# DanMcGann/loam

Measured on AMD Instinct MI355X. Metric: scan-pair registrations/sec (64x1024 Ouster), higher is better.
Workload: dtype f64; 1 GPU; batch of 1024 independent 64x1024 scan pairs per GPU (BASELINE configs[2]/[3]); step = extractFeatures x2 + registerFeatures per pair, inputs resident in HBM; pairs_per_gpu=1024, scan=64x1024, seed=20240311, input_scalar=f64, arithmetic=f64 (float input is widened on load)

## Files before the change

include/loamx.h:

```cpp
#ifndef LOAMX_H_
#define LOAMX_H_

#include <stddef.h>
#include <stdint.h>

#ifdef __cplusplus
extern "C" {
#endif

typedef struct loamx_ctx loamx_ctx;

enum {
  LOAMX_OK = 0,
  LOAMX_ERR_SCAN_SIZE = 1,
  LOAMX_ERR_BAD_PARAM = 2,
  LOAMX_ERR_HIP = 3,
  LOAMX_ERR_CAPACITY = 4,
  LOAMX_ERR_UNSUPPORTED = 5,
  LOAMX_ERR_NO_DEVICE = 6,
  LOAMX_ERR_COMM = 7
};

typedef struct {
  uint64_t scan_lines;
// ... 65 lines not shown
int loamx_ctx_synchronize(loamx_ctx* ctx);
int loamx_ctx_extract_counters(loamx_ctx* ctx, uint64_t* tie_replays, uint64_t* scan_fallbacks);
enum {
  LOAMX_ROUTE_SPLIT_CURV = 1u << 0,
  LOAMX_ROUTE_CURV2 = 1u << 1,
  LOAMX_ROUTE_CURV_V1 = 1u << 2,
  LOAMX_ROUTE_CURV_GENERIC = 1u << 3,
  LOAMX_ROUTE_ROWS = 1u << 4,
  LOAMX_ROUTE_ROWS_CH11 = 1u << 5,
  LOAMX_ROUTE_ROWS_PASS2 = 1u << 6,
  LOAMX_ROUTE_ROWS_LIST16 = 1u << 7,
  LOAMX_ROUTE_MIS = 1u << 8,
  LOAMX_ROUTE_MIS_4LINES = 1u << 9,
  LOAMX_ROUTE_MIS_TWO = 1u << 10,
  LOAMX_ROUTE_MIS_CONST_W = 1u << 11,
  LOAMX_ROUTE_ARGMAX4 = 1u << 12,
  LOAMX_ROUTE_ARGMAX1 = 1u << 13,
  LOAMX_ROUTE_FUSED_COMPACT = 1u << 14,
  LOAMX_ROUTE_COMPACT = 1u << 15,
  LOAMX_ROUTE_FUSED_EXTRACT = 1u << 16,
  LOAMX_ROUTE_FUSED_ROWS = 1u << 17,
  LOAMX_ROUTE_BOXES = 1u << 18,
  LOAMX_ROUTE_ROWS_R_SHIFT = 20,
  LOAMX_ROUTE_ROWS_CH_SHIFT = 24
};
int loamx_ctx_last_extract_route(loamx_ctx* ctx, uint32_t* bits);
enum {
  LOAMX_WALK_NONE = 0,
  LOAMX_WALK_FLAT = 1,
  LOAMX_WALK_TILED_BY_COUNT = 2,
  LOAMX_WALK_TILED_BY_TILES = 3
};
typedef struct {
  uint32_t iterations, termination;
  uint32_t use_moments;
  uint32_t mom_ref_on;
  double mom_ref[7];
  uint32_t tiles;
  uint32_t live_tiles;
  uint64_t edge_stride, planar_stride;
  uint32_t n_se, n_sp;
  uint32_t walk;
  uint32_t listed_total;
  double s0max, v2max;
  uint32_t sweep_chunk, edge_cache, list_cache, flat_cache;
  uint32_t* tile_counts;
  size_t tile_counts_cap;
} loamx_solve_census;
int loamx_ctx_last_solve_census(loamx_ctx* ctx, size_t pair, loamx_solve_census* out);
enum { LOAMX_ASSOC_SEARCH_NONE = 0, LOAMX_ASSOC_SEARCH_BRUTE = 1, LOAMX_ASSOC_SEARCH_GRID = 2 };
enum { LOAMX_ASSOC_LEFTOVER_NONE = 0, LOAMX_ASSOC_LEFTOVER_LEFT = 1, LOAMX_ASSOC_LEFTOVER_COOP = 2 };
#define LOAMX_ASSOC_REASON_WIDE 0x80000000u
#define LOAMX_ASSOC_REASON_TIED 0x40000000u
typedef struct {
  uint32_t n_src, n_tgt;
  uint64_t stride;
  uint32_t km;
  uint32_t search;
  uint32_t mixed_launch;
  uint32_t one_stage;
  uint32_t leftover_kernel;
  uint32_t rest_blocks, coop_blocks;
  uint32_t rest_spread, left_spread;
  uint32_t lean_set;
  double origin[3], h;
  int32_t nx, ny, nz;
  uint32_t n_points;
  uint32_t verified, unverified, queued_words;
  uint32_t queued, queued_plain, queued_wide, queued_tied;
  uint32_t rest_searched;
  uint32_t listed;
  uint32_t leftover_finished;
  uint32_t exact;
  uint32_t late;
  uint32_t* entry_query;
  uint32_t* entry_reason;
  int32_t* count_after_rest;
  int32_t* count_before_fit;
  size_t entries_cap;
  uint32_t* late_query;
  size_t late_cap;
} loamx_assoc_census;
int loamx_ctx_last_assoc_census(loamx_ctx* ctx, int which_kind, loamx_assoc_census* out);
int loamx_ctx_set_option(loamx_ctx* ctx, const char* name, int value);
int loamx_ctx_get_option(loamx_ctx* ctx, const char* name, int* value);


int loamx_compute_curvature(loamx_ctx* ctx, const double* xyz, size_t n_points, const loamx_lidar_params* lidar,
                            const loamx_fe_params* fe, double* curvature_out);
int loamx_compute_valid_points(loamx_ctx* ctx, const double* xyz, size_t n_points,
                               const loamx_lidar_params* lidar, const loamx_fe_params* fe, uint8_t* mask_out);
int loamx_extract_features(loamx_ctx* ctx, const double* xyz, size_t n_points, const loamx_lidar_params* lidar,
                           const loamx_fe_params* fe, uint32_t* edge_idx, size_t edge_cap, size_t* n_edge,
                           uint32_t* planar_idx, size_t planar_cap, size_t* n_planar);
int loamx_compute_curvature_f32(loamx_ctx* ctx, const float* xyz, size_t n_points, const loamx_lidar_params* lidar,
                                const loamx_fe_params* fe, double* curvature_out);
int loamx_compute_valid_points_f32(loamx_ctx* ctx, const float* xyz, size_t n_points,
                                   const loamx_lidar_params* lidar, const loamx_fe_params* fe, uint8_t* mask_out);
int loamx_extract_features_f32(loamx_ctx* ctx, const float* xyz, size_t n_points, const loamx_lidar_params* lidar,
                               const loamx_fe_params* fe, uint32_t* edge_idx, size_t edge_cap, size_t* n_edge,
                               uint32_t* planar_idx, size_t planar_cap, size_t* n_planar);
int loamx_register_features(loamx_ctx* ctx, const double* src_edge, size_t n_src_edge, const double* src_planar,
                            size_t n_src_planar, const double* tgt_edge, size_t n_tgt_edge,
                            const double* tgt_planar, size_t n_tgt_planar, const double init_pose[7],
                            const loamx_reg_params* reg, loamx_reg_result* result, loamx_reg_detail* detail);

typedef struct loamx_target_index loamx_target_index;
int loamx_target_index_create(loamx_ctx* ctx, const double* tgt_edge, size_t n_tgt_edge, const double* tgt_planar,
                              size_t n_tgt_planar, const loamx_reg_params* reg, loamx_target_index** out);
void loamx_target_index_destroy(loamx_ctx* ctx, loamx_target_index* index);
int loamx_target_index_insert(loamx_ctx* ctx, loamx_target_index* index, const double* edge, size_t n_edge,
                              const double* planar, size_t n_planar);
int loamx_target_index_stats(const loamx_target_index* index, uint64_t* full_builds, uint64_t* merges);
int loamx_target_index_size(const loamx_target_index* index, size_t* n_edge, size_t* n_planar);
enum {
  LOAMX_INDEX_BUILD_NONE = 0,
  LOAMX_INDEX_BUILD_PACKED = 1,
  LOAMX_INDEX_BUILD_SINGLE = 2,
  LOAMX_INDEX_BUILD_BIG = 3
};
enum { LOAMX_INDEX_OP_NONE = 0, LOAMX_INDEX_OP_FULL_BUILD = 1, LOAMX_INDEX_OP_MERGE = 2 };
typedef struct {
  uint64_t n, capacity;
  double origin[3], h, inv_h;
  int32_t nx, ny, nz;
  uint32_t n_points;
  uint32_t build;
  uint32_t table_valid;
  uint64_t table_entries;
  uint32_t lds_passes;
  uint32_t scan_tiles;
  uint32_t last_op, reserved;
  uint64_t full_builds, merges;
  uint32_t* cell_start;
  size_t cell_start_cap;
  double* xyz;
  uint32_t* orig;
  size_t points_cap;
  float* rel;
  size_t rel_cap;
} loamx_index_census;
int loamx_target_index_census(loamx_ctx* ctx, const loamx_target_index* index, int which_set, loamx_index_census* out);
int loamx_register_features_indexed(loamx_ctx* ctx, const loamx_target_index* index, const double* src_edge,
                                    size_t n_src_edge, const double* src_planar, size_t n_src_planar,
                                    const double init_pose[7], const loamx_reg_params* reg, loamx_reg_result* result,
                                    loamx_reg_detail* detail);


int loamx_target_index_points(loamx_ctx* ctx, const loamx_target_index* index, int which_set, size_t first, size_t count,
                              double* xyz_out);
int loamx_voxel_filter_dev(loamx_ctx* ctx, const double* d_xyz, size_t n, const double pose[7], double leaf, double* d_xyz_out,
                           uint32_t* d_src_idx, uint32_t* d_n_out);
int loamx_target_index_insert_filtered(loamx_ctx* ctx, loamx_target_index* index, const double* edge, size_t n_edge,
                                       const double* planar, size_t n_planar, const double world_T_scan[7], double edge_leaf,
                                       double planar_leaf, size_t* n_edge_added, size_t* n_planar_added);
int loamx_target_index_crop(loamx_ctx* ctx, loamx_target_index* index, const double lo[3], const double hi[3],
                            size_t* n_edge_removed, size_t* n_planar_removed);


int loamx_fit_lines(loamx_ctx* ctx, const double* points, size_t n_sets, size_t k, double* lines_out, double* cond_out);
int loamx_fit_planes(loamx_ctx* ctx, const double* points, size_t n_sets, size_t k, double* planes_out, double* avg_dist_out);
int loamx_knn_search(loamx_ctx* ctx, const loamx_target_index* index, int which_set, const double* queries, size_t n_queries,
                     size_t k, double max_dist, uint32_t* indices_out, uint32_t* counts_out);
typedef struct {
  uint32_t* edge_nn_count;
  uint32_t* edge_nn_idx;
// ... 316 lines not shown
```

loam_amd/capi.py:

```python
import collections
import ctypes as C
import os

import numpy as np

from . import build as _build

OK, ERR_SCAN_SIZE, ERR_BAD_PARAM, ERR_HIP, ERR_CAPACITY, ERR_UNSUPPORTED, ERR_NO_DEVICE, ERR_COMM = range(8)
CONVERGED, MAX_ITER, INSUFFICIENT_ASSOCIATIONS = 0, 1, 2
K_CURVATURE, K_SELECT, K_COMPACT, K_GRID, K_ASSOC, K_SWEEP, K_LM, K_MOMENT, K_KNN_PLANE, K_EXTRACT_FUSED, K_INFORMATION, K_CLOUD_ACCUMULATE, K_CLOUD_ACCUMULATE_PLAIN, K_CLOUD_LIST, K_CLOUD_EMIT, K_COUNT = range(16)


class LidarParams(C.Structure):
    _fields_ = [("scan_lines", C.c_uint64), ("points_per_line", C.c_uint64), ("min_range", C.c_double),
                ("max_range", C.c_double)]


class FeatureExtractionParams(C.Structure):
    _fields_ = [("neighbor_points", C.c_uint64), ("number_sectors", C.c_uint64),
                ("max_edge_feats_per_sector", C.c_uint64), ("max_planar_feats_per_sector", C.c_uint64),
                ("edge_feat_threshold", C.c_double), ("planar_feat_threshold", C.c_double),
                ("occlusion_thresh", C.c_double), ("parallel_thresh", C.c_double)]

    def __init__(self, *a, **kw):
# ... 148 lines not shown
            if not 0 <= getattr(self, name) <= 0xFFFFFFFF:
                raise ValueError(f"PlaceParams: {name} does not fit 32 bits")
        return PlaceParamsStruct(self.n_rings, self.n_sectors, self.max_range, self.z_offset, self.z_scale)


PLACE_MATCH_DTYPE = np.dtype([("id", np.uint32), ("shift", np.uint32), ("key_dist", np.uint64), ("distance", np.float64)])
PLACE_NO_ID = 0xFFFFFFFF


class CloudMapParamsStruct(C.Structure):
    _fields_ = [("leaf", C.c_double), ("min_range", C.c_double), ("max_range", C.c_double)]


class CloudMapParams:

    def __init__(self, leaf=None, min_range=None, max_range=None):
        d = CloudMapParamsStruct()
        load().loamx_default_cloud_map_params(C.byref(d))
        self.leaf = d.leaf if leaf is None else float(leaf)
        self.min_range = d.min_range if min_range is None else float(min_range)
        self.max_range = d.max_range if max_range is None else float(max_range)

    def struct(self):
        return CloudMapParamsStruct(float(self.leaf), float(self.min_range), float(self.max_range))


CLOUD_MAP_STATS_DTYPE = np.dtype([(n, np.uint64) for n in ("voxels", "points_offered", "points_used", "invalid", "range", "outside", "overflow")])


class PgoParamsStruct(C.Structure):
    _fields_ = [("max_iterations", C.c_uint32), ("max_pcg_iterations", C.c_uint32), ("pcg_tolerance", C.c_double),
                ("initial_lambda", C.c_double), ("cost_tolerance", C.c_double), ("step_tolerance", C.c_double),
                ("huber_delta", C.c_double)]


class PgoParams:
    FIELDS = tuple(f[0] for f in PgoParamsStruct._fields_)

    def __init__(self, **kw):
        d = PgoParamsStruct()
        load().loamx_pgo_default_params(C.byref(d))
        for name in self.FIELDS:
            setattr(self, name, getattr(d, name))
        for name, v in kw.items():
            if name not in self.FIELDS:
                raise TypeError(f"PgoParams has no field {name}")
            setattr(self, name, v)

    def struct(self):
        for name in self.FIELDS[:2]:
            if not 0 <= int(getattr(self, name)) <= 0xFFFFFFFF:
                raise ValueError(f"PgoParams: {name} does not fit 32 bits")
        return PgoParamsStruct(int(self.max_iterations), int(self.max_pcg_iterations), *(float(getattr(self, n)) for n in self.FIELDS[2:]))


PGO_EDGE_DTYPE = np.dtype([("a", np.uint32), ("b", np.uint32), ("a_T_b", np.float64, 7), ("information", np.float64, (6, 6))])
PGO_SUMMARY_DTYPE = np.dtype([("initial_cost", np.float64), ("final_cost", np.float64), ("lambda", np.float64), ("max_update", np.float64),
                              ("iterations", np.uint32), ("accepted", np.uint32), ("pcg_iterations", np.uint32),
                              ("termination", np.uint32), ("n_bad_edges", np.uint32), ("reserved", np.uint32)])
PGO_LINEARIZATION_DTYPE = np.dtype([("e", np.float64, 6), ("chi2", np.float64), ("weight", np.float64), ("A", np.float64, (6, 6)),
                                    ("B", np.float64, (6, 6))])
PGO_TERMINATIONS = ("COST_CONVERGED", "STEP_CONVERGED", "MAX_ITERATIONS", "LAMBDA_OVERFLOW", "NOTHING_TO_DO", "BAD_INPUT")
(PGO_COST_CONVERGED, PGO_STEP_CONVERGED, PGO_MAX_ITERATIONS, PGO_LAMBDA_OVERFLOW, PGO_NOTHING_TO_DO, PGO_BAD_INPUT) = range(6)


EXPORTS = [
    "loamx_default_fe_params", "loamx_default_reg_params", "loamx_status_string", "loamx_last_error",
    "loamx_ctx_create", "loamx_ctx_destroy", "loamx_ctx_set_stream", "loamx_ctx_synchronize",
    "loamx_compute_curvature", "loamx_compute_valid_points", "loamx_extract_features", "loamx_register_features",
    "loamx_target_index_create", "loamx_target_index_destroy", "loamx_register_features_indexed",
    "loamx_edge_capacity", "loamx_planar_capacity", "loamx_extract_features_batch_dev",
    "loamx_register_features_batch_dev", "loamx_register_scan_pairs_dev", "loamx_register_scan_pairs",
    "loamx_register_scan_pairs_f32", "loamx_ctx_enable_kernel_timing",
    "loamx_ctx_reset_kernel_stats", "loamx_ctx_get_kernel_stats", "loamx_kernel_name", "loamx_synth_pair_pose",
    "loamx_synth_scan_host", "loamx_synth_scan_pairs_dev", "loamx_dev_alloc", "loamx_dev_free",
    "loamx_copy_to_device", "loamx_copy_to_host",
    "loamx_compute_curvature_f32", "loamx_compute_valid_points_f32", "loamx_extract_features_f32",
    "loamx_extract_features_batch_dev_f32", "loamx_register_scan_pairs_dev_f32",
    "loamx_target_index_insert", "loamx_target_index_size", "loamx_target_index_census",
    "loamx_shard_range", "loamx_comm_get_unique_id", "loamx_comm_create", "loamx_comm_wrap", "loamx_comm_destroy",
    "loamx_comm_info", "loamx_gather_results_dev", "loamx_comm_barrier", "loamx_comm_stats", "loamx_ctx_extract_counters",
    "loamx_ctx_set_option", "loamx_ctx_get_option", "loamx_ctx_last_extract_route", "loamx_ctx_last_solve_census",
    "loamx_ctx_last_assoc_census",
    "loamx_fit_lines", "loamx_fit_planes", "loamx_knn_search", "loamx_associate", "loamx_target_index_stats",
    "loamx_register_scan_sequence_dev", "loamx_register_scan_sequence_dev_f32", "loamx_register_scan_sequence",
    "loamx_register_scan_sequence_f32", "loamx_compose_trajectory_dev", "loamx_deskew_scans_dev", "loamx_deskew_scans_dev_f32",
    "loamx_deskew_launch_geometry",
    "loamx_target_index_points", "loamx_voxel_filter_dev", "loamx_target_index_insert_filtered", "loamx_target_index_crop",
    "loamx_registration_information", "loamx_registration_information_indexed", "loamx_registration_information_batch_dev",
    "loamx_register_scan_pairs_info_dev", "loamx_register_scan_pairs_info_dev_f32", "loamx_register_scan_sequence_info_dev",
    "loamx_register_scan_sequence_info_dev_f32",
    "loamx_default_organize_params", "loamx_scan_layout_create", "loamx_scan_layout_destroy", "loamx_scan_layout_tables",
    "loamx_organize_clouds_dev", "loamx_organize_clouds_dev_f32", "loamx_organize_cloud", "loamx_organize_cloud_f32",
    "loamx_default_place_params", "loamx_place_db_create", "loamx_place_db_destroy", "loamx_place_db_sector_dirs", "loamx_place_db_size",
    "loamx_place_descriptors_dev", "loamx_place_descriptors_dev_f32", "loamx_place_db_add_dev", "loamx_place_db_read",
    "loamx_place_search_dev", "loamx_place_descriptor", "loamx_place_descriptor_f32", "loamx_place_search",
    "loamx_pgo_default_params", "loamx_pose_graph_optimize_dev", "loamx_pose_graph_optimize", "loamx_pose_graph_linearize",
    "loamx_pose_graph_edges_from_results_dev",
    "loamx_default_cloud_map_params", "loamx_cloud_map_create", "loamx_cloud_map_destroy", "loamx_cloud_map_clear",
    "loamx_cloud_map_add_clouds_dev", "loamx_cloud_map_add_clouds_dev_f32", "loamx_cloud_map_emit_dev", "loamx_cloud_map_stats_read",
    "loamx_cloud_map_add_cloud", "loamx_cloud_map_add_cloud_f32", "loamx_cloud_map_emit", "loamx_cloud_map_claims_read",
]

ROUTE_BITS = ("SPLIT_CURV", "CURV2", "CURV_V1", "CURV_GENERIC", "ROWS", "ROWS_CH11", "ROWS_PASS2", "ROWS_LIST16", "MIS", "MIS_4LINES",
              "MIS_TWO", "MIS_CONST_W", "ARGMAX4", "ARGMAX1", "FUSED_COMPACT", "COMPACT", "FUSED_EXTRACT", "FUSED_ROWS", "BOXES")


class ExtractRoute:

    def __init__(self, bits):
        self.bits = int(bits)
        self.names = frozenset(n for i, n in enumerate(ROUTE_BITS) if self.bits >> i & 1)
        self.rows_R = self.bits >> 20 & 7
        self.rows_ch = self.bits >> 24 & 63

    def __contains__(self, name):
        if name not in ROUTE_BITS:
            raise KeyError(name)
        return name in self.names

    def __repr__(self):
        return "ExtractRoute(%s%s)" % ("|".join(n for n in ROUTE_BITS if n in self.names),
                                       ", R=%d ch=%d" % (self.rows_R, self.rows_ch) if "ROWS" in self.names else "")


class SolveCensusStruct(C.Structure):
    _fields_ = [("iterations", C.c_uint32), ("termination", C.c_uint32), ("use_moments", C.c_uint32), ("mom_ref_on", C.c_uint32),
                ("mom_ref", C.c_double * 7), ("tiles", C.c_uint32), ("live_tiles", C.c_uint32),
                ("edge_stride", C.c_uint64), ("planar_stride", C.c_uint64), ("n_se", C.c_uint32), ("n_sp", C.c_uint32),
                ("walk", C.c_uint32), ("listed_total", C.c_uint32), ("s0max", C.c_double), ("v2max", C.c_double),
                ("sweep_chunk", C.c_uint32), ("edge_cache", C.c_uint32), ("list_cache", C.c_uint32), ("flat_cache", C.c_uint32),
                ("tile_counts", C.POINTER(C.c_uint32)), ("tile_counts_cap", C.c_size_t)]


WALK_NONE, WALK_FLAT, WALK_TILED_BY_COUNT, WALK_TILED_BY_TILES = 0, 1, 2, 3
WALK_NAMES = ("none", "flat", "tiled-by-count", "tiled-by-tiles")
SolveCensus = collections.namedtuple(
    "SolveCensus", "iterations termination use_moments mom_ref_on mom_ref tiles live_tiles edge_stride planar_stride n_se n_sp walk "
                   "listed_total s0max v2max sweep_chunk edge_cache list_cache flat_cache tile_counts")


class AssocCensusStruct(C.Structure):
    _fields_ = ([("n_src", C.c_uint32), ("n_tgt", C.c_uint32), ("stride", C.c_uint64)] +
                [(n, C.c_uint32) for n in ("km", "search", "mixed_launch", "one_stage", "leftover_kernel", "rest_blocks", "coop_blocks",
                                           "rest_spread", "left_spread", "lean_set")] +
                [("origin", C.c_double * 3), ("h", C.c_double), ("nx", C.c_int32), ("ny", C.c_int32), ("nz", C.c_int32)] +
                [(n, C.c_uint32) for n in ("n_points", "verified", "unverified", "queued_words", "queued", "queued_plain", "queued_wide",
                                           "queued_tied", "rest_searched", "listed", "leftover_finished", "exact", "late")] +
                [("entry_query", C.POINTER(C.c_uint32)), ("entry_reason", C.POINTER(C.c_uint32)),
                 ("count_after_rest", C.POINTER(C.c_int32)), ("count_before_fit", C.POINTER(C.c_int32)), ("entries_cap", C.c_size_t),
                 ("late_query", C.POINTER(C.c_uint32)), ("late_cap", C.c_size_t)])


ASSOC_SEARCH_NONE, ASSOC_SEARCH_BRUTE, ASSOC_SEARCH_GRID = 0, 1, 2
ASSOC_LEFTOVER_NONE, ASSOC_LEFTOVER_LEFT, ASSOC_LEFTOVER_COOP = 0, 1, 2
ASSOC_REASON_WIDE, ASSOC_REASON_TIED = 0x80000000, 0x40000000
ASSOC_CENSUS_SCALARS = ("n_src n_tgt stride km search mixed_launch one_stage leftover_kernel rest_blocks coop_blocks rest_spread left_spread "
                        "lean_set h nx ny nz n_points verified unverified queued_words queued queued_plain queued_wide queued_tied "
                        "rest_searched listed leftover_finished exact late").split()
AssocCensus = collections.namedtuple("AssocCensus", ASSOC_CENSUS_SCALARS + ["origin", "entry_query", "entry_reason", "count_after_rest",
                                                                            "count_before_fit", "late_query"])


class IndexCensusStruct(C.Structure):
    _fields_ = [("n", C.c_uint64), ("capacity", C.c_uint64), ("origin", C.c_double * 3), ("h", C.c_double), ("inv_h", C.c_double),
                ("nx", C.c_int32), ("ny", C.c_int32), ("nz", C.c_int32), ("n_points", C.c_uint32),
# ... 49 lines not shown
    lib.loamx_compute_valid_points_f32.argtypes = [vp, fp, C.c_size_t, C.POINTER(LidarParams),
                                                   C.POINTER(FeatureExtractionParams), C.POINTER(C.c_uint8)]
    lib.loamx_extract_features_f32.argtypes = [vp, fp, C.c_size_t, C.POINTER(LidarParams),
                                               C.POINTER(FeatureExtractionParams), u32p, C.c_size_t,
                                               C.POINTER(C.c_size_t), u32p, C.c_size_t, C.POINTER(C.c_size_t)]
    lib.loamx_register_features.argtypes = [vp, dp, C.c_size_t, dp, C.c_size_t, dp, C.c_size_t, dp, C.c_size_t, dp,
                                            C.POINTER(RegistrationParams), C.POINTER(RegResult),
                                            C.POINTER(RegDetail)]
    lib.loamx_target_index_create.argtypes = [vp, dp, C.c_size_t, dp, C.c_size_t, C.POINTER(RegistrationParams), C.POINTER(vp)]
    lib.loamx_target_index_insert.argtypes = [vp, vp, dp, C.c_size_t, dp, C.c_size_t]
    lib.loamx_target_index_size.argtypes = [vp, C.POINTER(C.c_size_t), C.POINTER(C.c_size_t)]
    lib.loamx_target_index_stats.argtypes = [vp, C.POINTER(C.c_uint64), C.POINTER(C.c_uint64)]
    lib.loamx_target_index_points.argtypes = [vp, vp, C.c_int, C.c_size_t, C.c_size_t, dp]
    lib.loamx_target_index_census.argtypes = [vp, vp, C.c_int, C.POINTER(IndexCensusStruct)]
    lib.loamx_voxel_filter_dev.argtypes = [vp, vp, C.c_size_t, dp, C.c_double, vp, vp, vp]
    lib.loamx_target_index_insert_filtered.argtypes = [vp, vp, dp, C.c_size_t, dp, C.c_size_t, dp, C.c_double, C.c_double,
                                                       C.POINTER(C.c_size_t), C.POINTER(C.c_size_t)]
    lib.loamx_target_index_crop.argtypes = [vp, vp, dp, dp, C.POINTER(C.c_size_t), C.POINTER(C.c_size_t)]
    lib.loamx_target_index_destroy.argtypes = [vp, vp]
    lib.loamx_target_index_destroy.restype = None
    lib.loamx_register_features_indexed.argtypes = [vp, vp, dp, C.c_size_t, dp, C.c_size_t, dp, C.POINTER(RegistrationParams),
                                                    C.POINTER(RegResult), C.POINTER(RegDetail)]
    lib.loamx_edge_capacity.restype = C.c_size_t
    lib.loamx_edge_capacity.argtypes = [C.POINTER(LidarParams), C.POINTER(FeatureExtractionParams)]
    lib.loamx_planar_capacity.restype = C.c_size_t
    lib.loamx_planar_capacity.argtypes = [C.POINTER(LidarParams), C.POINTER(FeatureExtractionParams)]
    lib.loamx_extract_features_batch_dev.argtypes = [vp, vp, C.c_size_t, C.POINTER(LidarParams),
                                                     C.POINTER(FeatureExtractionParams), vp, vp, vp, vp, vp, vp]
    lib.loamx_extract_features_batch_dev_f32.argtypes = lib.loamx_extract_features_batch_dev.argtypes
    lib.loamx_register_features_batch_dev.argtypes = [vp, C.c_size_t, vp, vp, vp, vp, vp, vp, vp, vp, C.c_size_t,
                                                      C.c_size_t, vp, C.POINTER(RegistrationParams), vp]
    lib.loamx_register_scan_pairs_dev.argtypes = [vp, vp, C.c_size_t, C.POINTER(LidarParams),
                                                  C.POINTER(FeatureExtractionParams), C.POINTER(RegistrationParams),
                                                  vp]
    lib.loamx_register_scan_pairs_dev_f32.argtypes = lib.loamx_register_scan_pairs_dev.argtypes
    lib.loamx_register_scan_pairs.argtypes = lib.loamx_register_scan_pairs_dev.argtypes
    lib.loamx_register_scan_pairs_f32.argtypes = lib.loamx_register_scan_pairs_dev.argtypes
    lib.loamx_register_scan_sequence_dev.argtypes = [vp, vp, C.c_size_t, C.POINTER(LidarParams),
                                                     C.POINTER(FeatureExtractionParams), C.POINTER(RegistrationParams),
                                                     vp, vp]
    lib.loamx_register_scan_sequence_dev_f32.argtypes = lib.loamx_register_scan_sequence_dev.argtypes
    lib.loamx_register_scan_sequence.argtypes = lib.loamx_register_scan_sequence_dev.argtypes
    lib.loamx_register_scan_sequence_f32.argtypes = lib.loamx_register_scan_sequence_dev.argtypes
    lib.loamx_compose_trajectory_dev.argtypes = [vp, vp, C.c_size_t, dp, vp]
    lib.loamx_deskew_scans_dev.argtypes = [vp, vp, C.c_size_t, C.POINTER(LidarParams), vp, C.c_double, vp]
    lib.loamx_deskew_scans_dev_f32.argtypes = lib.loamx_deskew_scans_dev.argtypes
    lib.loamx_deskew_launch_geometry.argtypes = [C.c_size_t, C.c_uint64, C.c_uint64, u32p]
    lib.loamx_ctx_enable_kernel_timing.argtypes = [vp, C.c_int]
    lib.loamx_ctx_reset_kernel_stats.argtypes = [vp]
    lib.loamx_ctx_get_kernel_stats.argtypes = [vp, C.POINTER(KernelStat)]
    lib.loamx_synth_pair_pose.argtypes = [C.c_uint64, C.c_uint64, dp]
    lib.loamx_synth_pair_pose.restype = None
    lib.loamx_synth_scan_host.argtypes = [C.c_uint64, C.c_uint64, C.c_uint32, C.c_uint32, C.c_uint32, C.c_double, dp]
    lib.loamx_synth_scan_host.restype = None
    lib.loamx_synth_scan_pairs_dev.argtypes = [vp, C.c_uint64, C.c_uint64, C.c_size_t, C.c_uint32, C.c_uint32,
                                               C.c_double, vp]
    lib.loamx_dev_alloc.argtypes = [vp, C.c_size_t, C.POINTER(vp)]
    lib.loamx_dev_free.argtypes = [vp, vp]
    lib.loamx_copy_to_device.argtypes = [vp, vp, vp, C.c_size_t]
    lib.loamx_copy_to_host.argtypes = [vp, vp, vp, C.c_size_t]
    szp = C.POINTER(C.c_size_t)
    lib.loamx_shard_range.argtypes = [C.c_size_t, C.c_int, C.c_int, szp, szp]
    lib.loamx_shard_range.restype = None
    lib.loamx_comm_get_unique_id.argtypes = [C.c_char_p]
    lib.loamx_comm_create.argtypes = [vp, C.c_char_p, C.c_int, C.c_int, C.POINTER(vp)]
    lib.loamx_comm_wrap.argtypes = [vp, vp, C.POINTER(vp)]
    lib.loamx_comm_destroy.argtypes = [vp]
    lib.loamx_comm_destroy.restype = None
    lib.loamx_comm_info.argtypes = [vp, C.POINTER(C.c_int), C.POINTER(C.c_int), C.POINTER(C.c_int)]
    lib.loamx_gather_results_dev.argtypes = [vp, vp, vp, C.c_size_t, C.c_size_t, vp]
    lib.loamx_comm_barrier.argtypes = [vp, vp, dp]
    lib.loamx_comm_stats.argtypes = [vp, C.POINTER(C.c_uint64)]
    lib.loamx_ctx_extract_counters.argtypes = [vp, C.POINTER(C.c_uint64), C.POINTER(C.c_uint64)]
    lib.loamx_fit_lines.argtypes = [vp, dp, C.c_size_t, C.c_size_t, dp, dp]
    lib.loamx_fit_planes.argtypes = [vp, dp, C.c_size_t, C.c_size_t, dp, dp]
    lib.loamx_knn_search.argtypes = [vp, vp, C.c_int, dp, C.c_size_t, C.c_size_t, C.c_double, vp, vp]
    lib.loamx_associate.argtypes = [vp, dp, C.c_size_t, dp, C.c_size_t, dp, C.c_size_t, dp, C.c_size_t, dp,
                                    C.POINTER(RegistrationParams), C.POINTER(AssocDump)]
    lib.loamx_ctx_set_option.argtypes = [vp, C.c_char_p, C.c_int]
    lib.loamx_ctx_get_option.argtypes = [vp, C.c_char_p, C.POINTER(C.c_int)]
    lib.loamx_ctx_last_extract_route.argtypes = [vp, C.POINTER(C.c_uint32)]
    lib.loamx_ctx_last_solve_census.argtypes = [vp, C.c_size_t, C.POINTER(SolveCensusStruct)]
    lib.loamx_ctx_last_assoc_census.argtypes = [vp, C.c_int, C.POINTER(AssocCensusStruct)]
    lib.loamx_registration_information.argtypes = [vp, dp, C.c_size_t, dp, C.c_size_t, dp, C.c_size_t, dp, C.c_size_t, dp,
                                                   C.POINTER(RegistrationParams), C.POINTER(RegInformation)]
    lib.loamx_registration_information_indexed.argtypes = [vp, vp, dp, C.c_size_t, dp, C.c_size_t, dp, C.POINTER(RegistrationParams),
                                                           C.POINTER(RegInformation)]
    lib.loamx_registration_information_batch_dev.argtypes = lib.loamx_register_features_batch_dev.argtypes
    lib.loamx_register_scan_pairs_info_dev.argtypes = lib.loamx_register_scan_pairs_dev.argtypes + [vp]
    lib.loamx_register_scan_pairs_info_dev_f32.argtypes = lib.loamx_register_scan_pairs_info_dev.argtypes
    lib.loamx_register_scan_sequence_info_dev.argtypes = lib.loamx_register_scan_sequence_dev.argtypes + [vp]
    lib.loamx_register_scan_sequence_info_dev_f32.argtypes = lib.loamx_register_scan_sequence_info_dev.argtypes
    lib.loamx_default_organize_params.argtypes = [C.POINTER(OrganizeParamsStruct)]
    lib.loamx_default_organize_params.restype = None
    lib.loamx_scan_layout_create.argtypes = [vp, C.POINTER(LidarParams), C.POINTER(OrganizeParamsStruct), C.POINTER(vp)]
    lib.loamx_scan_layout_destroy.argtypes = [vp, vp]
    lib.loamx_scan_layout_destroy.restype = None
    lib.loamx_scan_layout_tables.argtypes = [vp, dp, dp]
    lib.loamx_organize_clouds_dev.argtypes = [vp, vp, vp, C.c_size_t, vp, szp, C.c_size_t, vp, vp, vp]
    lib.loamx_organize_clouds_dev_f32.argtypes = lib.loamx_organize_clouds_dev.argtypes
    lib.loamx_organize_cloud.argtypes = [vp, vp, vp, C.c_size_t, vp, C.c_size_t, vp, vp, vp]
    lib.loamx_organize_cloud_f32.argtypes = lib.loamx_organize_cloud.argtypes
    lib.loamx_default_place_params.argtypes = [C.POINTER(PlaceParamsStruct)]
    lib.loamx_default_place_params.restype = None
    lib.loamx_place_db_create.argtypes = [vp, C.POINTER(PlaceParamsStruct), C.POINTER(vp)]
    lib.loamx_place_db_destroy.argtypes = [vp, vp]
    lib.loamx_place_db_destroy.restype = None
    lib.loamx_place_db_sector_dirs.argtypes = [vp, dp]
    lib.loamx_place_db_size.argtypes = [vp, szp]
    lib.loamx_place_descriptors_dev.argtypes = [vp, vp, vp, C.c_size_t, szp, C.c_size_t, vp]
    lib.loamx_place_descriptors_dev_f32.argtypes = lib.loamx_place_descriptors_dev.argtypes
    lib.loamx_place_db_add_dev.argtypes = [vp, vp, vp, C.c_size_t, u32p]
    lib.loamx_place_db_read.argtypes = [vp, vp, C.c_size_t, C.c_size_t, vp, vp, vp]
    lib.loamx_place_search_dev.argtypes = [vp, vp, vp, C.c_size_t, vp, C.c_uint32, vp]
    lib.loamx_place_descriptor.argtypes = [vp, vp, vp, C.c_size_t, C.c_size_t, vp]
    lib.loamx_place_descriptor_f32.argtypes = lib.loamx_place_descriptor.argtypes
    lib.loamx_place_search.argtypes = lib.loamx_place_search_dev.argtypes
    lib.loamx_default_cloud_map_params.argtypes = [C.POINTER(CloudMapParamsStruct)]
    lib.loamx_default_cloud_map_params.restype = None
    lib.loamx_cloud_map_create.argtypes = [vp, C.POINTER(CloudMapParamsStruct), C.c_size_t, C.POINTER(vp)]
    lib.loamx_cloud_map_destroy.argtypes = [vp, vp]
    lib.loamx_cloud_map_destroy.restype = None
    lib.loamx_cloud_map_clear.argtypes = [vp, vp]
    lib.loamx_cloud_map_add_clouds_dev.argtypes = [vp, vp, vp, C.c_size_t, szp, C.c_size_t, vp]
    lib.loamx_cloud_map_add_clouds_dev_f32.argtypes = lib.loamx_cloud_map_add_clouds_dev.argtypes
    lib.loamx_cloud_map_emit_dev.argtypes = [vp, vp, C.c_uint32, vp, vp, vp, C.c_size_t, vp]
    lib.loamx_cloud_map_stats_read.argtypes = [vp, vp, vp]
    lib.loamx_cloud_map_claims_read.argtypes = [vp, vp, C.POINTER(C.c_uint64)]
    lib.loamx_cloud_map_add_cloud.argtypes = [vp, vp, vp, C.c_size_t, C.c_size_t, vp]
    lib.loamx_cloud_map_add_cloud_f32.argtypes = lib.loamx_cloud_map_add_cloud.argtypes
    lib.loamx_cloud_map_emit.argtypes = [vp, vp, C.c_uint32, vp, vp, vp, C.c_size_t, szp]
    lib.loamx_pgo_default_params.argtypes = [C.POINTER(PgoParamsStruct)]
    lib.loamx_pgo_default_params.restype = None
    lib.loamx_pose_graph_optimize_dev.argtypes = [vp, vp, C.c_size_t, vp, vp, C.c_size_t, C.POINTER(PgoParamsStruct), vp]
    lib.loamx_pose_graph_optimize.argtypes = lib.loamx_pose_graph_optimize_dev.argtypes
    lib.loamx_pose_graph_linearize.argtypes = [vp, vp, C.c_size_t, vp, C.c_size_t, C.c_double, vp]
    lib.loamx_pose_graph_edges_from_results_dev.argtypes = [vp, vp, vp, C.c_size_t, C.c_uint32, vp]
    _lib = lib
    return lib


class LoamxError(RuntimeError):
    def __init__(self, status, message):
        super().__init__(message)
        self.status = status


DeskewGeometry = collections.namedtuple("DeskewGeometry", "col_blocks shares lines_per_share unroll")


def deskew_launch_geometry(n_scans, scan_lines, points_per_line):
    v = (C.c_uint32 * 4)()
    rc = load().loamx_deskew_launch_geometry(n_scans, scan_lines, points_per_line, v)
    if rc != OK:
        raise LoamxError(rc, "loamx_deskew_launch_geometry: " + load().loamx_status_string(rc).decode())
    return DeskewGeometry(*(int(x) for x in v))


def _dp(a):
    return a.ctypes.data_as(C.POINTER(C.c_double))


def _pts(a):
    a = np.ascontiguousarray(np.asarray(a, dtype=np.float64).reshape(-1, 3))
    return a

# ... 319 lines not shown
        p = C.c_void_p()
        ctx._check(ctx.lib.loamx_dev_alloc(ctx.h, nbytes, C.byref(p)))
        self.ptr = p.value

    def upload(self, arr):
        arr = np.ascontiguousarray(arr)
        assert arr.nbytes <= self.nbytes
        self.ctx._check(self.ctx.lib.loamx_copy_to_device(self.ctx.h, self.ptr, arr.ctypes.data, arr.nbytes))
        return self

    def download(self, dtype, count):
        out = np.empty(count, dtype=dtype)
        assert out.nbytes <= self.nbytes
        self.ctx._check(self.ctx.lib.loamx_copy_to_host(self.ctx.h, out.ctypes.data, self.ptr, out.nbytes))
        return out

    def free(self):
        if self.ptr:
            self.ctx.lib.loamx_dev_free(self.ctx.h, self.ptr)
            self.ptr = None


class Context:

    def __init__(self, device=0):
        self.lib = load()
        h = C.c_void_p()
        rc = self.lib.loamx_ctx_create(device, C.byref(h))
        if rc != OK:
            raise LoamxError(rc, "loamx_ctx_create: " + self.lib.loamx_status_string(rc).decode() +
                             " (libloamx has no CPU fallback)")
        self.h = h

    def close(self):
        if getattr(self, "h", None):
            self.lib.loamx_ctx_destroy(self.h)
            self.h = None

    def __del__(self):
        try:
            self.close()
        except Exception:
            pass

    def _check(self, rc):
        if rc != OK:
            msg = self.lib.loamx_last_error(self.h).decode() or self.lib.loamx_status_string(rc).decode()
            raise LoamxError(rc, msg)

    def set_stream(self, hip_stream_handle):
        self._check(self.lib.loamx_ctx_set_stream(self.h, hip_stream_handle))

    def synchronize(self):
        self._check(self.lib.loamx_ctx_synchronize(self.h))

    def set_option(self, name, value=1):
        self._check(self.lib.loamx_ctx_set_option(self.h, name.encode(), int(value)))

    def get_option(self, name):
        v = C.c_int(0)
        self._check(self.lib.loamx_ctx_get_option(self.h, name.encode(), C.byref(v)))
        return v.value

    def extract_counters(self):
        a, b = C.c_uint64(0), C.c_uint64(0)
        self._check(self.lib.loamx_ctx_extract_counters(self.h, C.byref(a), C.byref(b)))
        return a.value, b.value

    def last_extract_route(self):
        v = C.c_uint32(0)
        self._check(self.lib.loamx_ctx_last_extract_route(self.h, C.byref(v)))
        return ExtractRoute(v.value)

    def last_solve_census(self, pair=0):
        v = SolveCensusStruct()
        self._check(self.lib.loamx_ctx_last_solve_census(self.h, pair, C.byref(v)))
        counts = np.zeros(max(1, v.live_tiles), dtype=np.uint32)
        v.tile_counts, v.tile_counts_cap = counts.ctypes.data_as(C.POINTER(C.c_uint32)), v.live_tiles
        self._check(self.lib.loamx_ctx_last_solve_census(self.h, pair, C.byref(v)))
        return SolveCensus(v.iterations, v.termination, v.use_moments, v.mom_ref_on, np.array(list(v.mom_ref)), v.tiles, v.live_tiles,
                           v.edge_stride, v.planar_stride, v.n_se, v.n_sp, v.walk, v.listed_total, v.s0max, v.v2max, v.sweep_chunk,
                           v.edge_cache, v.list_cache, v.flat_cache, counts[:v.live_tiles].copy())

    def last_assoc_census(self, kind):
        kind = {"edge": 0, "plane": 1}.get(kind, kind)
        v = AssocCensusStruct()
        self._check(self.lib.loamx_ctx_last_assoc_census(self.h, kind, C.byref(v)))
        q = int(v.queued)
        eq, er = np.zeros(max(1, q), dtype=np.uint32), np.zeros(max(1, q), dtype=np.uint32)
        ar, bf = np.zeros(max(1, q), dtype=np.int32), np.zeros(max(1, q), dtype=np.int32)
        v.entry_query, v.entry_reason = eq.ctypes.data_as(C.POINTER(C.c_uint32)), er.ctypes.data_as(C.POINTER(C.c_uint32))
        v.count_after_rest, v.count_before_fit = ar.ctypes.data_as(C.POINTER(C.c_int32)), bf.ctypes.data_as(C.POINTER(C.c_int32))
        v.entries_cap = q
        nl = int(v.late)
        lq = np.zeros(max(1, nl), dtype=np.uint32)
        v.late_query, v.late_cap = lq.ctypes.data_as(C.POINTER(C.c_uint32)), nl
        self._check(self.lib.loamx_ctx_last_assoc_census(self.h, kind, C.byref(v)))
        return AssocCensus(*[getattr(v, n) for n in ASSOC_CENSUS_SCALARS], np.array(list(v.origin)), eq[:q].copy(), er[:q].copy(),
                           ar[:q].copy(), bf[:q].copy(), lq[:nl].copy())

    def alloc(self, nbytes):
        return DeviceBuffer(self, nbytes)

    def compute_curvature(self, xyz, lidar, fe=None):
        fe = fe or FeatureExtractionParams()
        xyz = _scan(xyz)
        out = np.empty(len(xyz))
        fn = self.lib.loamx_compute_curvature_f32 if xyz.dtype == np.float32 else self.lib.loamx_compute_curvature
        self._check(fn(self.h, _xyzp(xyz), len(xyz), C.byref(lidar), C.byref(fe), _dp(out)))
        return out

    def compute_valid_points(self, xyz, lidar, fe=None):
        fe = fe or FeatureExtractionParams()
        xyz = _scan(xyz)
        out = np.empty(len(xyz), dtype=np.uint8)
        fn = self.lib.loamx_compute_valid_points_f32 if xyz.dtype == np.float32 else self.lib.loamx_compute_valid_points
        self._check(fn(self.h, _xyzp(xyz), len(xyz), C.byref(lidar), C.byref(fe), out.ctypes.data_as(C.POINTER(C.c_uint8))))
        return out.astype(bool)

    def extract_features(self, xyz, lidar, fe=None):
        fe = fe or FeatureExtractionParams()
        xyz = _scan(xyz)
        ecap = max(1, self.lib.loamx_edge_capacity(C.byref(lidar), C.byref(fe)))
        pcap = max(1, self.lib.loamx_planar_capacity(C.byref(lidar), C.byref(fe)))
        e = np.empty(ecap, dtype=np.uint32)
        p = np.empty(pcap, dtype=np.uint32)
        ne, npl = C.c_size_t(0), C.c_size_t(0)
        u32p = C.POINTER(C.c_uint32)
        fn = self.lib.loamx_extract_features_f32 if xyz.dtype == np.float32 else self.lib.loamx_extract_features
        self._check(fn(self.h, _xyzp(xyz), len(xyz), C.byref(lidar), C.byref(fe), e.ctypes.data_as(u32p), ecap, C.byref(ne),
                       p.ctypes.data_as(u32p), pcap, C.byref(npl)))
        return e[:ne.value].copy(), p[:npl.value].copy()

    def register_features(self, src_edge, src_planar, tgt_edge, tgt_planar, init_pose=None, reg=None,
                          want_detail=False):
        reg = reg or RegistrationParams()
        arrs = [_pts(a) for a in (src_edge, src_planar, tgt_edge, tgt_planar)]
        init = np.ascontiguousarray([0, 0, 0, 1, 0, 0, 0] if init_pose is None else init_pose, dtype=np.float64)
        res = RegResult()
        detail = None
        if want_detail:
            mi = max(1, reg.max_iterations)
            info = (IterInfo * mi)()
            ce, cp = max(1, len(arrs[0])), max(1, len(arrs[1]))
            ep = np.zeros((mi, ce, 2), dtype=np.uint32)
            pp = np.zeros((mi, cp, 2), dtype=np.uint32)
            nep = np.zeros(mi, dtype=np.uint32)
            npp = np.zeros(mi, dtype=np.uint32)
            u32p = C.POINTER(C.c_uint32)
            detail = RegDetail(info, 0, ep.ctypes.data_as(u32p), ce, nep.ctypes.data_as(u32p),
                               pp.ctypes.data_as(u32p), cp, npp.ctypes.data_as(u32p))
        self._check(self.lib.loamx_register_features(
            self.h, _dp(arrs[0]), len(arrs[0]), _dp(arrs[1]), len(arrs[1]), _dp(arrs[2]), len(arrs[2]),
            _dp(arrs[3]), len(arrs[3]), _dp(init), C.byref(reg), C.byref(res),
            C.byref(detail) if detail is not None else None))
        pose = np.array(list(res.pose))
        if want_detail:
            d = dict(iterations=[dict(target_T_source_init=np.array(list(info[i].target_T_source_init)),
                                      estimate_update=np.array(list(info[i].estimate_update)),
                                      n_edge=info[i].n_edge_associations, n_plane=info[i].n_plane_associations,
                                      edge_pairs=ep[i, :nep[i]].copy(), plane_pairs=pp[i, :npp[i]].copy())
                                 for i in range(detail.n_iter_info)])
            return pose, res.termination, res.iterations, d
        return pose, res.termination, res.iterations

    def fit_lines(self, points):
# ... 394 lines not shown
```

loam_amd/csrc/api_core.hip:

```cpp
#include "api_host.h"
#include "synth.h"

using namespace loamx;

namespace loamx {
thread_local LaunchScope* g_launch_scope = nullptr;
int g_debug_sync = getenv("LOAMX_DEBUG_SYNC") ? 1 : 0;
thread_local uint32_t g_extract_route = 0;
}

namespace {

const char* kKernelNames[LOAMX_K_COUNT] = {"curvature_valid_kernel", "select_kernel", "compact_kernel",
                                           "grid_build_kernel",      "associate_kernel", "sweep_kernel",
                                           "lm_kernels",             "moment_kernel",    "knn_plane_kernel",
                                           "extract_fused_kernel",   "information_kernel", "cloud_accumulate_kernel",
                                           "cloud_accumulate_plain_kernel", "cloud_list_kernels", "cloud_emit_kernels"};

struct OptionName {
  const char* name;
  bool extract;
  uint32_t bit;
};
const OptionName kOptionNames[] = {
    {"FORCE_TIE_REPLAY", true, kFlagForceReplay}, {"FORCE_SCAN_GIVEUP", true, kFlagForceGiveUp}, {"CURV_V1", true, kFlagCurvV1},
    {"NO_FUSED_COMPACT", true, kFlagNoFusedCompact}, {"NO_MIS_SELECT", true, kFlagNoMisSelect}, {"FUSED_EXTRACT", true, kFlagFusedExtract},
    {"NO_ROW_SELECT", true, kFlagNoRowSelect}, {"FUSED_ROWS", true, kFlagFusedRows}, {"NO_SPLIT_CURV", true, kFlagNoSplitCurv}, {"STAGE_ALWAYS", true, kFlagStageAlways},
    {"NO_MOMENTS", false, kRegFlagNoMoments}, {"NO_PACKED_GRID", false, kRegFlagNoPackedGrid}, {"NO_BIG_GRID", false, kRegFlagNoBigGrid},
    {"NO_GRID_SIDE", false, kRegFlagNoGridSide}, {"DEBUG_POISON", false, kRegFlagPoison},
    {"QUEUE_TWO_STAGE", false, kRegFlagQueueTwoStage}, {"QUEUE_ONE_STAGE", false, kRegFlagQueueOneStage},
    {"NO_MIXED_ASSOC", false, kRegFlagNoMixedAssoc}, {"FORCE_RCCL", false, kRegFlagForceRccl},
    {"NO_COOP_LEFT", false, kRegFlagNoCoopLeft}, {"NO_REF_MOMENTS", false, kRegFlagNoRefMoments},
    {"NO_EXTRACT_BOXES", false, kRegFlagNoExtractBoxes}, {"CHECK_FINITE", false, kRegFlagCheckFinite},
    {"NO_SMALL_SETS", false, kRegFlagNoSmallSets}, {"FORCE_LATE_VERIFY", false, kRegFlagForceLate},
    {"NO_LIVE_DEAL", false, kRegFlagNoLiveDeal}, {"NO_CLOUDMAP_COMBINE", false, kRegFlagNoCloudmapCombine}};

}

namespace loamx {

int fail(loamx_ctx* ctx, int code, const std::string& msg) {
  if (ctx) ctx->last_error = msg;
  return code;
}

int ensure(loamx_ctx* ctx, Buf& b, size_t bytes) {
  if (bytes == 0) bytes = 8;
  if (b.cap >= bytes) return LOAMX_OK;
  if (b.p) {
    HIP_TRY(ctx, hipStreamSynchronize(ctx->stream));
    HIP_TRY(ctx, hipFree(b.p));
    b.p = nullptr, b.cap = 0;
  }
  HIP_TRY(ctx, hipMalloc(&b.p, bytes));
  b.cap = bytes;
  return LOAMX_OK;
}
int ensure(loamx_ctx* ctx, int id, size_t bytes) { return ensure(ctx, ctx->ws[id], bytes); }

const char* const kNonFiniteMsg = "non-finite coordinate in the input (the reference's behaviour is undefined there)";
bool host_all_finite(const void* p, bool f32, size_t n_scalars) {
  if (!p) return true;
  if (f32) {
    const float* v = static_cast<const float*>(p);
    float acc = 0.0f;
    for (size_t i = 0; i < n_scalars; i++) acc += v[i] * 0.0f;
    return acc == 0.0f;
  }
  const double* v = static_cast<const double*>(p);
  double acc = 0.0;
  for (size_t i = 0; i < n_scalars; i++) acc += v[i] * 0.0;
  return acc == 0.0;
}

hipEvent_t take_event(loamx_ctx* ctx) {
  if (!ctx->event_pool.empty()) {
    hipEvent_t e = ctx->event_pool.back();
    ctx->event_pool.pop_back();
    return e;
  }
  hipEvent_t e = nullptr;
  (void)hipEventCreate(&e);
  return e;
}

int finite_begin(loamx_ctx* ctx) {
  ENSURE(ctx, WS_FINITE_FLAG, 16);
  untimed(ctx);
  HIP_TRY(ctx, hipMemsetAsync(ctx->ws[WS_FINITE_FLAG].p, 0, 16, ctx->stream));
  return LOAMX_OK;
}
void finite_add(loamx_ctx* ctx, const void* d_pts, bool f32, const uint32_t* d_n, size_t n_sets, size_t stride, uint32_t pitch) {
  if (d_pts && n_sets && stride) launch_check_finite(d_pts, f32, d_n, n_sets, stride, pitch, static_cast<uint32_t*>(ctx->ws[WS_FINITE_FLAG].p), ctx->stream);
}
int finite_end(loamx_ctx* ctx) {
  uint32_t bad = 0;
  HIP_TRY(ctx, hipMemcpyAsync(&bad, ctx->ws[WS_FINITE_FLAG].p, 4, hipMemcpyDeviceToHost, ctx->stream));
  HIP_TRY(ctx, hipStreamSynchronize(ctx->stream));
  return bad ? fail(ctx, LOAMX_ERR_BAD_PARAM, kNonFiniteMsg) : LOAMX_OK;
}
int dev_check_finite(loamx_ctx* ctx, const void* d_pts, bool f32, const uint32_t* d_n, size_t n_sets, size_t stride, uint32_t pitch, bool force) {
  if ((!force && !(ctx->reg_flags & kRegFlagCheckFinite)) || !d_pts || n_sets == 0 || stride == 0) return LOAMX_OK;
  int rc = finite_begin(ctx);
  if (rc != LOAMX_OK) return rc;
  finite_add(ctx, d_pts, f32, d_n, n_sets, stride, pitch);
  return finite_end(ctx);
}

int check_finite_scalars(loamx_ctx* ctx, const double* d, size_t n) {
  int rc = finite_begin(ctx);
  if (rc != LOAMX_OK) return rc;
  launch_check_finite_scalars(d, n, static_cast<uint32_t*>(ctx->ws[WS_FINITE_FLAG].p), ctx->stream);
  return finite_end(ctx);
}

// ... 367 lines not shown
```

loam_amd/csrc/api_host.h:

```cpp
#pragma once
#include <math.h>
#include <stdio.h>
#include <stdlib.h>
#include <string.h>

#include <mutex>
#include <string>
#include <type_traits>
#include <utility>
#include <vector>

#include "loamx_internal.h"

namespace loamx {

enum WsId {
  WS_XYZ = 0, WS_CURV, WS_MASK,
  WS_SORT_SCRATCH, WS_SORT_SCRATCH_SRC, WS_NASSOC, WS_STATE, WS_PARTIALS, WS_MOM_PARTIALS, WS_MOMENTS, WS_FLAGGED_LIST, WS_FLAGGED_COUNT,
  WS_LINE_TOT, WS_EXTRACT_EVENTS, WS_BOX, WS_FINITE_FLAG, WS_COUNTERS, WS_ITERINFO, WS_STREAM_IN0, WS_STREAM_IN1, WS_STREAM_RES,
  WS_FIT_IN, WS_FIT_OUT, WS_FCOUNTS, WS_RESULTS, WS_INIT, WS_STREAM_INIT,
  WS_VOX_TABLE, WS_MAP_WORDS, WS_INFO_PARTIALS, WS_INFO, WS_LIVE,
  WS_ORG_WINNER, WS_ORG_RANGE, WS_ORG_CELL, WS_ORG_COUNTS, WS_ORG_IN, WS_ORG_RINGS, WS_ORG_OUT,
  WS_PLACE_TABLE, WS_PLACE_QKEYS, WS_PLACE_QNORMS, WS_PLACE_CAND_A, WS_PLACE_CAND_B, WS_PLACE_MATCH, WS_PLACE_IN, WS_PLACE_OUT,
  WS_PGO_WORK, WS_PGO_POSES, WS_PGO_FIXED, WS_PGO_EDGES, WS_PGO_OUT,
  WS_CLOUD_IN, WS_CLOUD_POSE, WS_CLOUD_OUT,
  WS_COUNT
};
enum WsKindId {
  WSK_STAGE = 0, WSK_CNT, WSK_IDX, WSK_N, WSK_XYZ,
  WSK_GRID_DESC, WSK_CELLS, WSK_SORTED, WSK_REL, WSK_SGRID_DESC, WSK_SCELLS, WSK_SSORTED, WSK_ASSOC, WSK_NN, WSK_RNN, WSK_NEAREST,
  WSK_REST, WSK_EXACT, WSK_DUMP, WSK_SRC, WSK_TGT, WSK_MAP_TMP, WSK_MAP_OUT, WSK_CENSUS,
  WSK_COUNT
};

struct Buf {
  void* p = nullptr;
  size_t cap = 0;
};

struct PendingEvent {
  int kernel;
  hipEvent_t e0, e1;
  double bytes;
  bool own_e0;
};

}

struct loamx_ctx {
  int device = 0;
  hipStream_t own_stream = nullptr, stream = nullptr;
  bool max_counts_clean = false;
  hipStream_t aux_stream = nullptr;
  hipEvent_t ev_fork = nullptr, ev_mid = nullptr, ev_join = nullptr;
  hipEvent_t ev_counts = nullptr;
  hipStream_t aux2_stream = nullptr;
  hipEvent_t ev_join2 = nullptr;
  std::string last_error;
  loamx::Buf ws[loamx::WS_COUNT];
  loamx::Buf wsk[loamx::WSK_COUNT][2];
  uint32_t* h_pinned = nullptr;
  bool timing = false;
  std::vector<loamx::PendingEvent> pending;
  std::vector<hipEvent_t> event_pool;
  hipEvent_t tail_event = nullptr;
  bool tail_fresh = false;
  loamx_kernel_stat stats[LOAMX_K_COUNT] = {};

  uint32_t extract_flags = 0;
  uint32_t reg_flags = 0;
  int map_cells_log2 = 0;
  int stream_chunk_pairs = 0;
  hipStream_t copy_stream = nullptr;
  hipEvent_t ev_up[2] = {nullptr, nullptr}, ev_free[2] = {nullptr, nullptr};

  uint32_t last_extract_route = 0;
  loamx::RegBatch last_solve_batch = {};
  uint32_t last_solve_flags = 0;
  bool last_solve_valid = false;
  struct AssocCensusKept {
    loamx_assoc_census c;
    std::vector<uint32_t> entry;
    std::vector<int32_t> after_rest, before_fit;
    std::vector<uint32_t> late;
  } last_assoc_census[2];
  bool last_assoc_census_valid = false;

  unsigned long long sweep_slots_base[2] = {0, 0};
  unsigned long long features_base = 0;
  std::mutex mu;
};

struct loamx_target_index {
  loamx::GridDesc* desc[2] = {nullptr, nullptr};
  uint32_t* cells[2] = {nullptr, nullptr};
  loamx::GridPoint* sorted[2] = {nullptr, nullptr};
  float* rel[2] = {nullptr, nullptr};
  double* pts[2] = {nullptr, nullptr};
  size_t n[2] = {0, 0};
  size_t cap[2] = {0, 0};
  double radius[2] = {0, 0};
  uint32_t* counts = nullptr;
  void* scratch = nullptr;
  uint32_t cells_cap[2] = {0, 0};
  size_t cells_alloc[2] = {0, 0}, scratch_alloc = 0;
  loamx::GridPoint* sorted2[2] = {nullptr, nullptr};
  float* rel2[2] = {nullptr, nullptr};
  size_t n_at_build[2] = {0, 0};
  bool grid_valid[2] = {false, false};
  uint64_t full_builds = 0, merges = 0;
  loamx::GridBuildForm build_form[2] = {{0u, 0u, 0u}, {0u, 0u, 0u}};
  bool table_valid[2] = {false, false};
  uint32_t last_op[2] = {0u, 0u};
  uint64_t kind_builds[2] = {0, 0}, kind_merges[2] = {0, 0};
  loamx::VoxelTable vox[2] = {{nullptr, nullptr, 0u}, {nullptr, nullptr, 0u}};
  double vox_leaf[2] = {0, 0};
  size_t vox_n[2] = {0, 0};
  bool vox_valid[2] = {false, false};
};

namespace loamx {

int fail(loamx_ctx* ctx, int code, const std::string& msg);

#define HIP_TRY(ctx, expr)                                                                          \
  do {                                                                                              \
    hipError_t e_ = (expr);                                                                         \
    if (e_ != hipSuccess)                                                                           \
      return fail(ctx, LOAMX_ERR_HIP, std::string(#expr) + ": " + hipGetErrorString(e_));           \
  } while (0)

int ensure(loamx_ctx* ctx, Buf& b, size_t bytes);
int ensure(loamx_ctx* ctx, int id, size_t bytes);
#define ENSURE(ctx, id, bytes)                       \
  do {                                               \
    int rc_ = ensure(ctx, id, bytes);                \
    if (rc_ != LOAMX_OK) return rc_;                 \
  } while (0)

template <typename T>
T* wsp(loamx_ctx* ctx, int id) {
  return reinterpret_cast<T*>(ctx->ws[id].p);
}
template <typename T>
T* wskp(loamx_ctx* ctx, int id, int kind) {
  return reinterpret_cast<T*>(ctx->wsk[id][kind].p);
}

int check_launch(loamx_ctx* ctx, const char* what);
#define CHECK_LAUNCH(ctx, what)                      \
  do {                                               \
    int rc_ = check_launch(ctx, what);               \
    if (rc_ != LOAMX_OK) return rc_;                 \
  } while (0)

struct ApiLock {
  std::lock_guard<std::mutex> guard;
  explicit ApiLock(loamx_ctx* ctx) : guard(ctx->mu) {}
};
#define API_LOCK(ctx)                                \
  if (!ctx) return LOAMX_ERR_BAD_PARAM;              \
  loamx::ApiLock api_lock_(ctx)
#define API_ENTER(ctx)                               \
  API_LOCK(ctx);                                     \
  HIP_TRY(ctx, hipSetDevice(ctx->device))

hipEvent_t take_event(loamx_ctx* ctx);
// ... 98 lines not shown
```

loam_amd/csrc/api_register.hip:

```cpp
#include "api_host.h"

using namespace loamx;

namespace {

int enqueue_association(loamx_ctx* ctx, const RegBatch& B, const RegConfig& C, uint32_t what = kAssocEdges | kAssocPlanes,
                        AssocCensusRun* census = nullptr) {
  hipStream_t s = ctx->stream;
  {
    TimedScope t(ctx, LOAMX_K_ASSOC, 0.0);
    const bool side = (size_t)B.n_pairs * B.kind[kPlane].assoc_blocks >= 128;
    PendingEvent knn{};
    LaunchScope knn_ls{nullptr, nullptr, true};
    if (ctx->timing) {
      knn.kernel = LOAMX_K_KNN_PLANE, knn.bytes = 0.0, knn.own_e0 = true;
      knn.e0 = take_event(ctx), knn.e1 = take_event(ctx);
      knn_ls = LaunchScope{knn.e0, knn.e1, true};
    }
    launch_associate(B, C, s, side ? ctx->aux_stream : nullptr, side ? ctx->aux2_stream : nullptr, ctx->ev_fork, ctx->ev_mid, ctx->ev_join,
                     ctx->ev_join2, ctx->timing ? &knn_ls : nullptr, what, census);
    if (ctx->timing) {
      if (knn_ls.first) ctx->event_pool.push_back(knn.e0), ctx->event_pool.push_back(knn.e1);
      else ctx->pending.push_back(knn);
    }
// ... 163 lines not shown

  if (prebuilt) {
    for (int k = 0; k < 2; k++) B.kind[k].grid = index_grid_set(prebuilt, k);
  }
  {
    TimedScope t(ctx, LOAMX_K_GRID, 0.0);
    const bool side = !(C.flags & kRegFlagNoGridSide) && ctx->aux_stream && !prebuilt && hipStreamWaitEvent(ctx->aux_stream, ctx->ev_counts, 0) == hipSuccess;
    if (!prebuilt) launch_grid_build_targets(B, C, s);
    launch_grid_build_sources(B, C, side ? ctx->aux_stream : s);
    if (side && hipEventRecord(ctx->ev_join, ctx->aux_stream) == hipSuccess) (void)hipStreamWaitEvent(s, ctx->ev_join, 0);
  }
  CHECK_LAUNCH(ctx, "grid_build_kernel");
  HIP_TRY(ctx, hipEventSynchronize(ctx->ev_counts));
  for (int k = 0; k < 2; k++) {
    B.kind[k].assoc_blocks = (ctx->h_pinned[16 + k] + 255u) / 256u;
    const uint32_t tmax = prebuilt ? (uint32_t)prebuilt->n[k] : ctx->h_pinned[18 + k], tmin = prebuilt ? tmax : ctx->h_pinned[20 + k];
    B.kind[k].knn_mode = tmin > tmax ? 0u : (tmin > kBruteMax ? 1u : (tmax <= kBruteMax ? 2u : 0u));
  }
  return LOAMX_OK;
}

int reg_dump(loamx_ctx* ctx, const RegBatch& B, const RegConfig& C, const loamx_assoc_dump* dump, const size_t n_src[2]) {
  if (B.n_pairs == 0) return LOAMX_OK;
  hipStream_t s = ctx->stream;
  if (B.n_pairs != 1) return fail(ctx, LOAMX_ERR_BAD_PARAM, "association dump: one pair at a time");
  RegBatch Bd = B;
  Bd.want_nn_counts = 1u;
  AssocCensusRun census = {};
  for (int kind = 0; kind < 2; kind++) {
    const size_t st = B.kind[kind].stride, bytes = 8 * sizeof(uint32_t) + 2 * st * sizeof(int32_t);
    ENSURE(ctx, ctx->wsk[WSK_CENSUS][kind], bytes);
    HIP_TRY(ctx, hipMemsetAsync(ctx->wsk[WSK_CENSUS][kind].p, 0, bytes, s));
    census.buf[kind].counts = wskp<uint32_t>(ctx, WSK_CENSUS, kind);
    census.buf[kind].after_rest = reinterpret_cast<int32_t*>(census.buf[kind].counts + 8);
    census.buf[kind].before_fit = census.buf[kind].after_rest + st;
  }
  int rc_a = enqueue_association(ctx, Bd, C, kAssocEdges | kAssocPlanes, &census);
  if (rc_a != LOAMX_OK) return rc_a;
  untimed(ctx);
  const size_t n[2] = {n_src[kEdge], n_src[kPlane]}, kq[2] = {(size_t)C.kind[kEdge].k, (size_t)C.kind[kPlane].k}, pw[2] = {6, 4};
  AssocDumpSet D[2] = {};
  for (int kind = 0; kind < 2; kind++) {
    const size_t bytes = n[kind] * (24 + 8 * pw[kind] + 4 + 4 * kq[kind] + 1) + 64;
    ENSURE(ctx, ctx->wsk[WSK_DUMP][kind], bytes);
    unsigned char* base = wskp<unsigned char>(ctx, WSK_DUMP, kind);
    HIP_TRY(ctx, hipMemsetAsync(base, 0, bytes, s));
    D[kind].moved = reinterpret_cast<double*>(base);
    D[kind].prim = D[kind].moved + 3 * n[kind];
    D[kind].nn_count = reinterpret_cast<uint32_t*>(D[kind].prim + pw[kind] * n[kind]);
    D[kind].nn_idx = D[kind].nn_count + n[kind];
    D[kind].valid = reinterpret_cast<uint8_t*>(D[kind].nn_idx + kq[kind] * n[kind]);
    if (n[kind] == 0) D[kind].nn_count = nullptr;
  }
  launch_assoc_dump(B, C, D, s);
  CHECK_LAUNCH(ctx, "assoc_dump_kernel");
  struct Out { void* host; const void* dev; size_t bytes; };
  const Out outs[10] = {
      {dump->edge_nn_count, D[0].nn_count, 4 * n[0]}, {dump->edge_nn_idx, D[0].nn_idx, 4 * kq[0] * n[0]}, {dump->edge_valid, D[0].valid, n[0]},
      {dump->edge_moved, D[0].moved, 24 * n[0]}, {dump->edge_lines, D[0].prim, 48 * n[0]},
      {dump->plane_nn_count, D[1].nn_count, 4 * n[1]}, {dump->plane_nn_idx, D[1].nn_idx, 4 * kq[1] * n[1]}, {dump->plane_valid, D[1].valid, n[1]},
      {dump->plane_moved, D[1].moved, 24 * n[1]}, {dump->plane_planes, D[1].prim, 32 * n[1]}};
  for (const Out& o : outs)
    if (o.host && o.bytes && o.dev) HIP_TRY(ctx, hipMemcpyAsync(o.host, o.dev, o.bytes, hipMemcpyDeviceToHost, s));
  if (dump->queue_lengths) HIP_TRY(ctx, hipMemcpyAsync(dump->queue_lengths, B.n_assoc + 2, 4 * sizeof(uint32_t), hipMemcpyDeviceToHost, s));
  HIP_TRY(ctx, hipStreamSynchronize(s));
  uint32_t na[8];
  HIP_TRY(ctx, hipMemcpy(na, B.n_assoc, sizeof(na), hipMemcpyDeviceToHost));
  for (int kind = 0; kind < 2; kind++) {
    const RegKind& K = B.kind[kind];
    const AssocCensusForm& F = census.form[kind];
    loamx_ctx::AssocCensusKept& keep = ctx->last_assoc_census[kind];
    loamx_assoc_census& c = keep.c;
    c = loamx_assoc_census{};
    GridDesc g;
    uint32_t counts[8];
    HIP_TRY(ctx, hipMemcpy(&g, K.grid.desc, sizeof(g), hipMemcpyDeviceToHost));
    if (F.km == 0u) g = GridDesc{};
    HIP_TRY(ctx, hipMemcpy(counts, census.buf[kind].counts, sizeof(counts), hipMemcpyDeviceToHost));
    c.n_src = (uint32_t)(n[kind] < K.stride ? n[kind] : K.stride), c.n_tgt = g.n_points, c.stride = K.stride;
    c.km = F.km, c.search = F.search, c.mixed_launch = F.mixed_launch, c.one_stage = F.one_stage, c.leftover_kernel = F.leftover_kernel;
    c.rest_blocks = F.rest_blocks, c.coop_blocks = F.coop_blocks;
    c.origin[0] = g.ox, c.origin[1] = g.oy, c.origin[2] = g.oz, c.h = g.h, c.nx = g.nx, c.ny = g.ny, c.nz = g.nz, c.n_points = g.n_points;
    c.verified = counts[0], c.unverified = counts[1], c.queued_words = counts[2];
    c.queued = na[2 + kind], c.listed = na[4 + kind], c.exact = counts[4], c.leftover_finished = counts[3] - counts[4], c.late = na[6 + kind];
    const uint32_t q = c.queued < K.stride ? c.queued : (uint32_t)K.stride;
    keep.entry.assign(q, 0u), keep.after_rest.assign(q, 0), keep.before_fit.assign(q, 0);
    if (q) {
      HIP_TRY(ctx, hipMemcpy(keep.entry.data(), K.rest, q * sizeof(uint32_t), hipMemcpyDeviceToHost));
      HIP_TRY(ctx, hipMemcpy(keep.after_rest.data(), census.buf[kind].after_rest, q * sizeof(int32_t), hipMemcpyDeviceToHost));
      HIP_TRY(ctx, hipMemcpy(keep.before_fit.data(), census.buf[kind].before_fit, q * sizeof(int32_t), hipMemcpyDeviceToHost));
    }
    uint32_t derived[4];
    assoc_census_derive(F, B.n_pairs, g, keep.entry.data(), q, na[4 + kind], derived);
    c.rest_spread = derived[0], c.left_spread = derived[1], c.lean_set = derived[2], c.rest_searched = derived[3];
    const uint32_t nl = c.late < K.stride ? c.late : (uint32_t)K.stride;
    keep.late.assign(nl, 0u);
    if (nl) HIP_TRY(ctx, hipMemcpy(keep.late.data(), K.exact + (K.stride - nl), nl * sizeof(uint32_t), hipMemcpyDeviceToHost));
    if (q || nl) {
      std::vector<GridPoint> sorted(c.n_src);
      HIP_TRY(ctx, hipMemcpy(sorted.data(), K.src_grid.sorted, (size_t)c.n_src * sizeof(GridPoint), hipMemcpyDeviceToHost));
      for (uint32_t t = 0; t < q; t++) {
        const uint32_t i = keep.entry[t] & 0x3FFFFFFFu;
        keep.entry[t] = (keep.entry[t] & ~0x3FFFFFFFu) | (i < c.n_src ? (sorted[i].orig & 0x3FFFFFFFu) : 0x3FFFFFFFu);
      }
      std::vector<uint32_t> tail(keep.late);
      for (uint32_t t = 0; t < nl; t++) {
        const uint32_t i = tail[nl - 1 - t];
        keep.late[t] = i < c.n_src ? sorted[i].orig : 0xFFFFFFFFu;
      }
    }
    for (uint32_t t = 0; t < q; t++) {
      if (keep.entry[t] & LOAMX_ASSOC_REASON_WIDE) c.queued_wide++;
      else if (keep.entry[t] & LOAMX_ASSOC_REASON_TIED) c.queued_tied++;
      else c.queued_plain++;
    }
  }
  ctx->last_assoc_census_valid = true;
  return LOAMX_OK;
}

int reg_information(loamx_ctx* ctx, const RegBatch& B, const RegConfig& C, InfoPartial* info_partials, loamx_reg_information* d_info, bool activate) {
  if (B.n_pairs == 0) return LOAMX_OK;
  hipStream_t s = ctx->stream;
  untimed(ctx);
  if (activate) launch_info_activate(B, s);
  const int rc_a = enqueue_association(ctx, B, C);
  if (rc_a != LOAMX_OK) return rc_a;
  {
    TimedScope t(ctx, LOAMX_K_INFORMATION, 0.0, true);
    launch_information(B, info_partials, d_info, s);
  }
  CHECK_LAUNCH(ctx, "information_kernel");
  return LOAMX_OK;
}

int reg_solve(loamx_ctx* ctx, const RegBatch& B, const RegConfig& C, loamx_reg_result* d_results, AfterAssocHook hook, void* hook_user) {
  if (B.n_pairs == 0) return LOAMX_OK;
  hipStream_t s = ctx->stream;
  ctx->last_solve_batch = B, ctx->last_solve_flags = C.flags, ctx->last_solve_valid = true;
  for (uint32_t it = 0; it < C.max_iterations; it++) {
    {
      const int rc_body = enqueue_icf_iteration(ctx, B, C, it, hook, hook_user);
      if (rc_body != LOAMX_OK) return rc_body;
    }
    if (it + 1 < C.max_iterations && it > (B.n_pairs >= 256 ? 1u : 0u)) {
      untimed(ctx);
      HIP_TRY(ctx, hipMemcpyAsync(ctx->h_pinned, B.live_count(it), sizeof(uint32_t), hipMemcpyDeviceToHost, s));
      launch_write_results(B, d_results, s);
      CHECK_LAUNCH(ctx, "write_results_kernel");
      HIP_TRY(ctx, hipStreamSynchronize(s));
      if (ctx->h_pinned[0] == 0) {
        ctx->max_counts_clean = true;
        return LOAMX_OK;
      }
    }
  }
  untimed(ctx);
  launch_write_results(B, d_results, s);
  CHECK_LAUNCH(ctx, "write_results_kernel");
  ctx->max_counts_clean = true;
  return LOAMX_OK;
}

}

namespace {
// ... 147 lines not shown
}

int loamx_registration_information(loamx_ctx* ctx, const double* src_edge, size_t n_se, const double* src_planar, size_t n_sp,
                                   const double* tgt_edge, size_t n_te, const double* tgt_planar, size_t n_tp, const double pose[7],
                                   const loamx_reg_params* reg, loamx_reg_information* info) {
  if (!info) return LOAMX_ERR_BAD_PARAM;
  return register_features_impl(ctx, nullptr, {{src_edge, src_planar}, {n_se, n_sp}}, {{tgt_edge, tgt_planar}, {n_te, n_tp}}, pose, reg,
                                HostOutput::to_info(info));
}

int loamx_registration_information_indexed(loamx_ctx* ctx, const loamx_target_index* index, const double* src_edge, size_t n_se,
                                           const double* src_planar, size_t n_sp, const double pose[7], const loamx_reg_params* reg,
                                           loamx_reg_information* info) {
  if (!index || !info) return LOAMX_ERR_BAD_PARAM;
  return register_features_impl(ctx, index, {{src_edge, src_planar}, {n_se, n_sp}}, {{nullptr, nullptr}, {0, 0}}, pose, reg,
                                HostOutput::to_info(info));
}

int loamx_ctx_last_solve_census(loamx_ctx* ctx, size_t pair, loamx_solve_census* out) {
  if (!out) return LOAMX_ERR_BAD_PARAM;
  API_ENTER(ctx);
  if (!ctx->last_solve_valid) return fail(ctx, LOAMX_ERR_BAD_PARAM, "no registration on this context to read (or its workspace has been handed on since)");
  const RegBatch& B = ctx->last_solve_batch;
  if (pair >= B.n_pairs) return fail(ctx, LOAMX_ERR_BAD_PARAM, "pair out of range");
  hipStream_t s = ctx->stream;
  untimed(ctx);
  HIP_TRY(ctx, hipStreamSynchronize(s));
  PairState S;
  uint32_t n_raw[2] = {0, 0};
  HIP_TRY(ctx, hipMemcpy(&S, B.state + pair, sizeof(S), hipMemcpyDeviceToHost));
  for (int k = 0; k < 2; k++) HIP_TRY(ctx, hipMemcpy(&n_raw[k], B.kind[k].n_src + pair * B.in_pitch, sizeof(uint32_t), hipMemcpyDeviceToHost));
  uint32_t* const counts_out = out->tile_counts;
  const size_t cap = counts_out ? out->tile_counts_cap : 0;
  *out = loamx_solve_census{};
  out->tile_counts = counts_out, out->tile_counts_cap = cap;
  out->iterations = S.iterations, out->termination = S.termination, out->use_moments = S.use_moments, out->mom_ref_on = S.mom_ref_on;
  for (int i = 0; i < 7; i++) out->mom_ref[i] = S.mom_ref[i];
  out->tiles = B.mom_blocks_per_pair * 4;
  out->edge_stride = B.kind[kEdge].stride, out->planar_stride = B.kind[kPlane].stride;
  out->n_se = n_raw[kEdge] < B.kind[kEdge].stride ? n_raw[kEdge] : (uint32_t)B.kind[kEdge].stride;
  out->n_sp = n_raw[kPlane] < B.kind[kPlane].stride ? n_raw[kPlane] : (uint32_t)B.kind[kPlane].stride;
  out->sweep_chunk = (uint32_t)kSweepChunk, out->edge_cache = kEdgeCache, out->list_cache = kListCache, out->flat_cache = kFlatCache;
  uint32_t live = 0;
  while (live < out->tiles && (size_t)(live / 4) * kSweepChunk < out->n_sp) live++;
  out->live_tiles = live;
  const bool lists = !(ctx->last_solve_flags & kRegFlagNoMoments) && (S.iterations >= 2u || S.mom_ref_on != 0u);
  if (!lists) return LOAMX_OK;
  double maxima[2];
  HIP_TRY(ctx, hipMemcpy(maxima, B.moments + pair * (size_t)(kMomSize + 2) + kMomSize, sizeof(maxima), hipMemcpyDeviceToHost));
  out->s0max = maxima[0], out->v2max = maxima[1];
  std::vector<uint32_t> cnt(live);
  if (live) HIP_TRY(ctx, hipMemcpy(cnt.data(), B.flagged_count + pair * (size_t)out->tiles, live * sizeof(uint32_t), hipMemcpyDeviceToHost));
  for (uint32_t t = 0; t < live; t++) {
    out->listed_total += cnt[t];
    if (t < cap) counts_out[t] = cnt[t];
  }
  out->walk = out->tiles > kListCache ? LOAMX_WALK_TILED_BY_TILES : (out->listed_total > kFlatCache ? LOAMX_WALK_TILED_BY_COUNT : LOAMX_WALK_FLAT);
  return LOAMX_OK;
}

int loamx_ctx_last_assoc_census(loamx_ctx* ctx, int which_kind, loamx_assoc_census* out) {
  if (!out) return LOAMX_ERR_BAD_PARAM;
  API_LOCK(ctx);
  if (which_kind != 0 && which_kind != 1) return fail(ctx, LOAMX_ERR_BAD_PARAM, "which_kind: 0 = edges, 1 = planes");
  if (!ctx->last_assoc_census_valid) return fail(ctx, LOAMX_ERR_BAD_PARAM, "no association dump on this context to read (or another call came after it)");
  const loamx_ctx::AssocCensusKept& keep = ctx->last_assoc_census[which_kind];
  uint32_t *const eq = out->entry_query, *const er = out->entry_reason;
  int32_t *const ar = out->count_after_rest, *const bf = out->count_before_fit;
  const size_t cap = out->entries_cap, lcap = out->late_cap;
  uint32_t* const lq = out->late_query;
  *out = keep.c;
  out->late_query = lq, out->late_cap = lcap;
  for (size_t t = 0; lq && t < keep.late.size() && t < lcap; t++) lq[t] = keep.late[t];
  out->entry_query = eq, out->entry_reason = er, out->count_after_rest = ar, out->count_before_fit = bf, out->entries_cap = cap;
  for (size_t t = 0; t < keep.entry.size() && t < cap; t++) {
    if (eq) eq[t] = keep.entry[t] & 0x3FFFFFFFu;
    if (er) er[t] = keep.entry[t] & (LOAMX_ASSOC_REASON_WIDE | LOAMX_ASSOC_REASON_TIED);
    if (ar) ar[t] = keep.after_rest[t];
    if (bf) bf[t] = keep.before_fit[t];
  }
  return LOAMX_OK;
}

int loamx_associate(loamx_ctx* ctx, const double* src_edge, size_t n_se, const double* src_planar, size_t n_sp, const double* tgt_edge,
                    size_t n_te, const double* tgt_planar, size_t n_tp, const double pose[7], const loamx_reg_params* reg,
                    loamx_assoc_dump* out) {
  if (!out) return LOAMX_ERR_BAD_PARAM;
  return register_features_impl(ctx, nullptr, {{src_edge, src_planar}, {n_se, n_sp}}, {{tgt_edge, tgt_planar}, {n_te, n_tp}}, pose, reg,
                                HostOutput::to_dump(out));
}

static int fit_sets(loamx_ctx* ctx, bool plane, const double* points, size_t n_sets, size_t k, double* prim_out, double* aux_out) {
  API_ENTER(ctx);
  if (n_sets == 0) return LOAMX_OK;
  if (!points || !prim_out) return fail(ctx, LOAMX_ERR_BAD_PARAM, "null argument");
  if (k < (plane ? 3u : 2u)) return fail(ctx, LOAMX_ERR_BAD_PARAM, plane ? "fitPlane needs k >= 3 points" : "fitLine needs k >= 2 points");
  if (k > (size_t)kFitMaxK) return fail(ctx, LOAMX_ERR_UNSUPPORTED, "point sets of more than 32 points are not supported by the fit kernels");
  if (n_sets > 0x7FFFFFFFull / 64) return fail(ctx, LOAMX_ERR_UNSUPPORTED, "too many point sets in one call");
  const size_t pw = plane ? 4 : 6;
  untimed(ctx);
  ENSURE(ctx, WS_FIT_IN, n_sets * k * 24);
  ENSURE(ctx, WS_FIT_OUT, n_sets * (pw + 1) * sizeof(double));
  double* d_prim = wsp<double>(ctx, WS_FIT_OUT);
  double* d_aux = d_prim + n_sets * pw;
  hipStream_t s = ctx->stream;
  HIP_TRY(ctx, hipMemcpyAsync(ctx->ws[WS_FIT_IN].p, points, n_sets * k * 24, hipMemcpyHostToDevice, s));
  {
    int rc = dev_check_finite(ctx, ctx->ws[WS_FIT_IN].p, false, nullptr, 1, n_sets * k, 1, true);
    if (rc != LOAMX_OK) return rc;
  }
  launch_fit_sets(plane, wsp<double>(ctx, WS_FIT_IN), n_sets, (int)k, d_prim, d_aux, s);
  CHECK_LAUNCH(ctx, "fit_sets_kernel");
  HIP_TRY(ctx, hipMemcpyAsync(prim_out, d_prim, n_sets * pw * sizeof(double), hipMemcpyDeviceToHost, s));
  if (aux_out) HIP_TRY(ctx, hipMemcpyAsync(aux_out, d_aux, n_sets * sizeof(double), hipMemcpyDeviceToHost, s));
  HIP_TRY(ctx, hipStreamSynchronize(s));
  return LOAMX_OK;
}

int loamx_fit_lines(loamx_ctx* ctx, const double* points, size_t n_sets, size_t k, double* lines_out, double* cond_out) {
  return fit_sets(ctx, false, points, n_sets, k, lines_out, cond_out);
}
int loamx_fit_planes(loamx_ctx* ctx, const double* points, size_t n_sets, size_t k, double* planes_out, double* avg_dist_out) {
  return fit_sets(ctx, true, points, n_sets, k, planes_out, avg_dist_out);
}

int loamx_knn_search(loamx_ctx* ctx, const loamx_target_index* index, int which_set, const double* queries, size_t n_queries, size_t k,
                     double max_dist, uint32_t* indices_out, uint32_t* counts_out) {
  if (!ctx || !index) return LOAMX_ERR_BAD_PARAM;
  API_ENTER(ctx);
  if (which_set != 0 && which_set != 1) return fail(ctx, LOAMX_ERR_BAD_PARAM, "which_set: 0 = edge points, 1 = planar points");
  if (index->n[which_set] != 0 && !index->grid_valid[which_set])
    return fail(ctx, LOAMX_ERR_BAD_PARAM, "the target index is inconsistent (an insert into it failed): insert again or build a new one");
  if (n_queries == 0) return LOAMX_OK;
  if (!queries || !indices_out || !counts_out) return fail(ctx, LOAMX_ERR_BAD_PARAM, "null argument");
  if (k == 0) {
    memset(counts_out, 0, n_queries * sizeof(uint32_t));
    return LOAMX_OK;
  }
  if (k > (size_t)kMaxK) return fail(ctx, LOAMX_ERR_UNSUPPORTED, "k > 16 neighbours not supported by the search kernels");
  if (n_queries > 0x7FFFFFFFull / 64) return fail(ctx, LOAMX_ERR_UNSUPPORTED, "too many queries in one call");
  untimed(ctx);
  ENSURE(ctx, WS_FIT_IN, n_queries * 24);
  ENSURE(ctx, WS_FIT_OUT, n_queries * (k + 1) * sizeof(uint32_t));
  uint32_t* d_idx = wsp<uint32_t>(ctx, WS_FIT_OUT);
  uint32_t* d_cnt = d_idx + n_queries * k;
  hipStream_t s = ctx->stream;
  HIP_TRY(ctx, hipMemcpyAsync(ctx->ws[WS_FIT_IN].p, queries, n_queries * 24, hipMemcpyHostToDevice, s));
  {
    int rc = dev_check_finite(ctx, ctx->ws[WS_FIT_IN].p, false, nullptr, 1, n_queries, 1, true);
    if (rc != LOAMX_OK) return rc;
  }
  launch_knn_queries(index_grid_set(index, which_set), wsp<double>(ctx, WS_FIT_IN), n_queries, (int)k, max_dist, d_idx, d_cnt, s);
  CHECK_LAUNCH(ctx, "knn_queries_kernel");
  HIP_TRY(ctx, hipMemcpyAsync(indices_out, d_idx, n_queries * k * sizeof(uint32_t), hipMemcpyDeviceToHost, s));
  HIP_TRY(ctx, hipMemcpyAsync(counts_out, d_cnt, n_queries * sizeof(uint32_t), hipMemcpyDeviceToHost, s));
  HIP_TRY(ctx, hipStreamSynchronize(s));
  return LOAMX_OK;
}

static int register_features_batch(loamx_ctx* ctx, size_t n_pairs, const double* d_src_edge, const uint32_t* d_n_src_edge,
                                   const double* d_src_planar, const uint32_t* d_n_src_planar, const double* d_tgt_edge,
                                   const uint32_t* d_n_tgt_edge, const double* d_tgt_planar, const uint32_t* d_n_tgt_planar,
                                   size_t edge_stride, size_t planar_stride, const double* d_init, const loamx_reg_params* reg,
                                   loamx_reg_result* d_results, loamx_reg_information* d_info) {
  API_ENTER(ctx);
  RegConfig C;
// ... 54 lines not shown
```

loam_amd/csrc/loamx_internal.h:

```cpp
#pragma once
#include <hip/hip_runtime.h>
#include <hip/hip_ext.h>
#include <stdint.h>
#include <stdio.h>

#include "../../include/loamx.h"
#include "extract_math.h"
#include "reg_math.h"
#include "organize_math.h"
#include "place_math.h"
#include "xcd_map.h"

namespace loamx {

struct LaunchScope {
  hipEvent_t start, stop;
  bool first;
};
extern thread_local LaunchScope* g_launch_scope;
extern int g_debug_sync;
template <typename F, typename... Args>
inline void launch_kernel_named(const char* name, F kernel, const dim3& grid, const dim3& block, size_t shmem, hipStream_t s, Args... args) {
  LaunchScope* sc = g_launch_scope;
  if (g_debug_sync) fprintf(stderr, "[loamx] launch %s grid %u x %u block %u\n", name, grid.x, grid.y, block.x), fflush(stderr);
// ... 13 lines not shown
constexpr int kMaxNeighborPoints = 16;
constexpr int kMaxLineWidth = 4096;

extern thread_local uint32_t g_extract_route;

struct ExtractStage {
  uint32_t* edge_stage;
  uint32_t* planar_stage;
  uint32_t* edge_cnt;
  uint32_t* planar_cnt;
};

struct ExtractFused {
  unsigned long long* line_tot;
  uint32_t fuse;
  const void* xyz;
  uint32_t f32;
  uint32_t* edge_idx;
  uint32_t* n_edge;
  double* edge_xyz;
  size_t edge_stride;
  uint32_t* planar_idx;
  uint32_t* n_planar;
  double* planar_xyz;
  size_t planar_stride;
  uint32_t* error;
  unsigned long long* events;
  unsigned long long* box_min;
  unsigned long long* box_max;
  uint32_t no_stage;
  const uint32_t* only_if;
};
__device__ __forceinline__ unsigned long long dbl_key(double v) {
  const unsigned long long u = (unsigned long long)__double_as_longlong(v);
  return (u >> 63) ? ~u : (u | 0x8000000000000000ull);
}
__device__ __forceinline__ double key_dbl(unsigned long long k) {
  return __longlong_as_double((long long)((k >> 63) ? (k & 0x7FFFFFFFFFFFFFFFull) : ~k));
}

void launch_curvature_valid(const void* d_xyz, bool f32, size_t n_scans, const ExtractParams& P, double* d_curv,
                            uint8_t* d_mask, hipStream_t s);
bool launch_select(const double* d_curv, const uint8_t* d_mask, size_t n_scans, const ExtractParams& P,
                   const ExtractStage& st, const ExtractFused* fz, hipStream_t s, bool* rows_ran = nullptr);
bool launch_select_takes_boxes(const ExtractParams& P);
bool launch_extract_fused(const void* d_xyz, bool f32, size_t n_scans, const ExtractParams& P, const ExtractStage& st,
                          const ExtractFused& fz, double* d_curv, uint8_t* d_mask, hipStream_t s);
bool launch_extract_rows_fused(const void* d_xyz, bool f32, size_t n_scans, const ExtractParams& P, const ExtractStage& st,
                               const ExtractFused& fz, double* d_curv, uint8_t* d_mask, hipStream_t s);
bool launch_extract_split_ok(const ExtractParams& P, size_t n_scans);
void launch_extract_init(unsigned long long* line_tot, size_t n_tot, unsigned long long* box_min, unsigned long long* box_max, size_t n_box,
                         hipStream_t s);
void launch_replay(const double* d_curv, const uint8_t* d_mask, size_t n_scans, const ExtractParams& P, const ExtractStage& st,
                   const ExtractFused& fz, hipStream_t s);
void launch_compact(const void* d_xyz, bool f32, size_t n_scans, const ExtractParams& P, const ExtractStage& st,
                    uint32_t* d_edge_idx, uint32_t* d_n_edge, double* d_edge_xyz, size_t edge_stride,
                    uint32_t* d_planar_idx, uint32_t* d_n_planar, double* d_planar_xyz, size_t planar_stride,
                    hipStream_t s, const uint32_t* only_if = nullptr, unsigned long long* fallback_counter = nullptr);

constexpr int kEdge = 0, kPlane = 1;
struct RegKindConfig {
  int k;
  double r;
  int min_pts;
  double pass;
};
struct RegConfig {
  RegKindConfig kind[2];
  double min_line_cond, max_avg_plane_dist;
  uint32_t max_iterations;
  double rot_thresh, pos_thresh;
  uint32_t min_associations;
  uint32_t flags;
};
constexpr uint32_t kRegFlagNoMoments = 1u;
constexpr uint32_t kRegFlagNoPackedGrid = 2u;
constexpr uint32_t kRegFlagNoBigGrid = 4u;
constexpr uint32_t kRegFlagNoGridSide = 8u;
constexpr uint32_t kRegFlagPoison = 16u;
constexpr uint32_t kRegFlagQueueTwoStage = 32u;
constexpr uint32_t kRegFlagQueueOneStage = 64u;
constexpr uint32_t kRegFlagForceRccl = 256u;
constexpr uint32_t kRegFlagNoCoopLeft = 512u;
constexpr uint32_t kRegFlagNoRefMoments = 1024u;
constexpr uint32_t kRegFlagNoSmallSets = 8192u;
constexpr uint32_t kRegFlagCheckFinite = 4096u;
constexpr uint32_t kRegFlagNoExtractBoxes = 2048u;
constexpr uint32_t kRegFlagNoMixedAssoc = 128u;
constexpr uint32_t kRegFlagNoLiveDeal = 32768u;
constexpr uint32_t kRegFlagForceLate = 16384u;

struct GridSet {
  GridDesc* desc;
  uint32_t* cell_start;
  GridPoint* sorted;
  size_t stride;
  float* rel;
  uint32_t cells_cap;
};

struct RegKind {
  size_t stride;
  const double* src;
  const uint32_t* n_src;
  const double* tgt;
  const uint32_t* n_tgt;
  GridSet grid;
  GridSet src_grid;
  uint32_t knn_mode;
  uint32_t assoc_blocks;
  double* rec;
  uint32_t* nn;
  uint32_t* rnn;
  uint32_t* nearest;
  uint32_t* rest;
  uint32_t* exact;
};

struct LiveLists {
  uint32_t iter;
  uint32_t n[2];
  uint32_t stamp[2];
  uint32_t pad[3];
};
constexpr uint32_t kLiveFirstIter = 2u;

struct PairState {
  double est[7];
  LmState lm;
  uint32_t active;
  uint32_t termination;
  uint32_t iterations;
  uint32_t first_sweep;
  uint32_t stream_planes;
  uint32_t use_moments;
  uint32_t mom_ref_on;
  double mom_ref[7];
};

constexpr int kSweepThreads = 256;
#ifndef LOAMX_SWEEP_ITEMS
#define LOAMX_SWEEP_ITEMS 16
#endif
constexpr int kSweepItems = LOAMX_SWEEP_ITEMS;
constexpr int kSweepChunk = kSweepThreads * kSweepItems;
constexpr uint32_t kEdgeCache = 320;
constexpr uint32_t kListCache = 64;
constexpr uint32_t kFlatCache = 192;

struct RegBatch {
  size_t n_pairs;
  uint32_t in_pitch;
  RegKind kind[2];
  const double* init;
  GridPoint* sort_scratch;
  GridPoint* sort_scratch_src;
  uint32_t* n_assoc;
  PairState* state;
  double* partials;
  double* mom_partials;
  double* moments;
  uint32_t mom_blocks_per_pair;
  uint32_t* flagged_list;
  uint32_t* flagged_count;
  uint32_t blocks_per_pair;
  uint32_t* n_active;
// ... 211 lines not shown
```

loam_amd/csrc/reg_math.h:

```cpp
#pragma once
#include <stdint.h>

#if defined(__HIPCC__)
#include <hip/hip_runtime.h>
#include <math.h>
#define LOAMX_HD __host__ __device__ __forceinline__
#else
#include <math.h>
#define LOAMX_HD inline
#endif

namespace loamx {

constexpr int kMaxK = 16;
constexpr double kDblMin = 2.2250738585072014e-308;
constexpr double kDblMax = 1.7976931348623157e308;
constexpr double kDblEps = 2.220446049250313e-16;

struct Vec3 {
  double x, y, z;
};
LOAMX_HD Vec3 v3(double x, double y, double z) { return Vec3{x, y, z}; }
LOAMX_HD Vec3 vadd(Vec3 a, Vec3 b) { return Vec3{a.x + b.x, a.y + b.y, a.z + b.z}; }
LOAMX_HD Vec3 vsub(Vec3 a, Vec3 b) { return Vec3{a.x - b.x, a.y - b.y, a.z - b.z}; }
// ... 701 lines not shown
  if (out > 1) return false;
  const double r2 = knn_radius_bound(max_dist);
  double sy2m = slab_dist(q.y, g.oy, g.h, cy - 1), sy2p = slab_dist(q.y, g.oy, g.h, cy + 1);
  double sz2m = slab_dist(q.z, g.oz, g.h, cz - 1), sz2p = slab_dist(q.z, g.oz, g.h, cz + 1);
  sy2m *= sy2m, sy2p *= sy2p, sz2m *= sz2m, sz2p *= sz2p;
  const int32_t xa = cx - 1 < 0 ? 0 : cx - 1, xb = cx + 1 > g.nx - 1 ? g.nx - 1 : cx + 1;
  uint32_t rb[9], re[9];
#pragma unroll
  for (int j = 0; j < 9; j++) {
    const int32_t iy = cy + (j % 3) - 1, iz = cz + (j / 3) - 1;
    const bool ok = xa <= xb && iy >= 0 && iy <= g.ny - 1 && iz >= 0 && iz <= g.nz - 1;
    const uint32_t row = ok ? (uint32_t)((iz * g.ny + iy) * g.nx) : 0u;
    rb[j] = ok ? cell_start_at(cell_start, row + (uint32_t)xa) : 0u;
    re[j] = ok ? cell_start_at(cell_start, row + (uint32_t)xb + 1u) : 0u;
  }
  uint32_t pre[10];
  pre[0] = 0u;
#pragma unroll
  for (int j = 0; j < 9; j++) {
    const double sy2 = j % 3 == 0 ? sy2m : (j % 3 == 1 ? 0.0 : sy2p), sz2 = j / 3 == 0 ? sz2m : (j / 3 == 1 ? 0.0 : sz2p);
    const bool in_reach = sy2 + sz2 <= r2;
    pre[j + 1] = pre[j] + ((in_reach && rb[j] < re[j]) ? re[j] - rb[j] : 0u);
  }
  const uint32_t total = pre[9];
  if (total > kRow16Cap) return false;
  KnnResult<KM> mine[NL];
#pragma unroll
  for (int v = 0; v < NL; v++) knn_init(mine[v]);
  for (uint32_t base = 0; base < total; base += (uint32_t)(kRow16Lanes * kRow16Batch)) {
#pragma unroll
    for (int v = 0; v < NL; v++) {
      uint32_t at[kRow16Batch];
      bool real[kRow16Batch];
#pragma unroll
      for (int u = 0; u < kRow16Batch; u++) {
        const uint32_t n = base + (uint32_t)(lane0 + v) + (uint32_t)(u * kRow16Lanes);
        real[u] = n < total;
        uint32_t p = 0u;
#pragma unroll
        for (int j = 0; j < 9; j++)
          if (n >= pre[j] && n < pre[j + 1]) p = rb[j] + (n - pre[j]);
        at[u] = p;
      }
      GridPoint t[kRow16Batch];
#pragma unroll
      for (int u = 0; u < kRow16Batch; u++)
        t[u] = *reinterpret_cast<const GridPoint*>(reinterpret_cast<const char*>(sp) + (uint32_t)(at[u] << 5));
#pragma unroll
      for (int u = 0; u < kRow16Batch; u++) {
        const double dx = q.x - t[u].x, dy = q.y - t[u].y, dz = q.z - t[u].z;
        const double d2 = dx * dx + dy * dy + dz * dz;
        if (real[u] && d2 <= mine[v].worst) knn_insert(mine[v], k, d2, at[u], t[u].orig);
      }
    }
  }
  knn_row16_select<KM, NL>(mine, k, r);
  kept = knn_finish(r, k, max_dist);
  if (!knn_done(g, q, k, max_dist, cx, cy, cz, r, 1)) {
    kept = 0;
    return false;
  }
  return true;
}

template <int KM>
LOAMX_HD int knn_search_keyed(const GridDesc& g, const uint32_t* __restrict__ cell_start, const GridPoint* __restrict__ sp,
                              Vec3 q, int k, double max_dist, double pass_max, uint32_t pos[KM], uint32_t* row_scratch,
                              int row_stride) {
#pragma unroll
  for (int j = 0; j < KM; j++) pos[j] = 0;
  if (g.n_points == 0 || k <= 0) return 0;
  if (k > KM) k = KM;
  const int32_t cx = grid_cell_coord(q.x, g.ox, g.inv_h);
  const int32_t cy = grid_cell_coord(q.y, g.oy, g.inv_h);
  const int32_t cz = grid_cell_coord(q.z, g.oz, g.inv_h);
  const int32_t out = grid_outside_distance(g, cx, cy, cz);
  if (max_dist > 0.0 && out >= 1 && (double)(out - 1) * g.h >= max_dist) return 0;
  KnnKeys<KM> c;
  knn_init(c, k, g.n_points);
  knn_rounds(g, cell_start, sp, q, k, max_dist, cx, cy, cz, c, out > 1 ? out : 1, row_scratch, row_stride);
  return knn_keys_finish(c, k, pass_max, pos);
}

template <int KM>
struct KnnKeys32 {
  uint32_t key[KM + 1];
};

LOAMX_HD uint32_t knn_umin(uint32_t a, uint32_t b) { return a < b ? a : b; }
LOAMX_HD uint32_t knn_umed3(uint32_t a, uint32_t b, uint32_t c) {
#if defined(__HIP_DEVICE_COMPILE__)
  uint32_t r;
  asm("v_med3_u32 %0, %1, %2, %3" : "=v"(r) : "v"(a), "v"(b), "v"(c));
  return r;
#else
  const uint32_t lo = a < b ? a : b, hi = a < b ? b : a;
  return c < lo ? lo : (c > hi ? hi : c);
#endif
}
LOAMX_HD uint32_t knn_f32_bits(float v) {
#if defined(__HIP_DEVICE_COMPILE__)
  return __float_as_uint(v);
#else
  uint32_t b;
  __builtin_memcpy(&b, &v, 4);
  return b;
#endif
}
LOAMX_HD float knn_bits_f32(uint32_t b) {
#if defined(__HIP_DEVICE_COMPILE__)
  return __uint_as_float(b);
#else
  float v;
  __builtin_memcpy(&v, &b, 4);
  return v;
#endif
}
template <int KM>
LOAMX_HD void knn_init(KnnKeys32<KM>& c, int k) {
#pragma unroll
  for (int j = 0; j <= KM; j++) c.key[j] = j < KM - k ? 0u : 0xFFFFFFFFu;
}
template <int KM>
LOAMX_HD void knn_key32_insert(KnnKeys32<KM>& c, uint32_t x) {
  uint32_t nk[KM + 1];
  nk[0] = knn_umin(c.key[0], x);
#pragma unroll
  for (int j = 1; j <= KM; j++) nk[j] = knn_umed3(c.key[j - 1], c.key[j], x);
#pragma unroll
  for (int j = 0; j <= KM; j++) c.key[j] = nk[j];
}
LOAMX_HD double knn_f32_err_unit(const GridDesc& g) {
  int32_t m = g.nx > g.ny ? g.nx : g.ny;
  m = m > g.nz ? m : g.nz;
  return 3.0 * 5.9604644775390625e-8 * ((double)(m + 2) * g.h);
}
template <int KM>
LOAMX_HD double knn_bound32(const KnnKeys32<KM>& c, double a, uint32_t imask) {
  const uint32_t kth = c.key[KM - 1];
  if (kth >= 0x7F800000u) return kDblMax;
  const double hi = (double)knn_bits_f32(kth | imask);
  return (hi + 3003.0 * a * a) * 1.002;
}

struct alignas(4) KnnF4 {
  float v[4];
};
template <int KM, bool MASK = true>
LOAMX_HD void knn_scan_batch_f32(KnnKeys32<KM>& c, float qx, float qy, float qz, const float* __restrict__ rel,
                                 uint32_t plane, uint32_t p, uint32_t n, uint32_t lidx, uint32_t imask) {
  const char* __restrict__ base = reinterpret_cast<const char*>(rel) + (uint32_t)(p << 2);
  const KnnF4 x = *reinterpret_cast<const KnnF4*>(base);
  const KnnF4 y = *reinterpret_cast<const KnnF4*>(base + (size_t)plane * 4);
  const KnnF4 z = *reinterpret_cast<const KnnF4*>(base + (size_t)plane * 8);
#if defined(LOAMX_KNN_STATS)
  g_cand += n < 4u ? n : 4u;
#endif
  uint32_t key[4];
#if defined(__HIP_DEVICE_COMPILE__)
  typedef float f2 __attribute__((ext_vector_type(2)));
  const f2 mqx = {-qx, -qx}, mqy = {-qy, -qy}, mqz = {-qz, -qz};
  const f2 x01 = {x.v[0], x.v[1]}, x23 = {x.v[2], x.v[3]}, y01 = {y.v[0], y.v[1]}, y23 = {y.v[2], y.v[3]};
  const f2 z01 = {z.v[0], z.v[1]}, z23 = {z.v[2], z.v[3]};
  const f2 dx01 = x01 + mqx, dx23 = x23 + mqx, dy01 = y01 + mqy, dy23 = y23 + mqy, dz01 = z01 + mqz, dz23 = z23 + mqz;
  f2 s01 = dx01 * dx01, s23 = dx23 * dx23;
  s01 = __builtin_elementwise_fma(dy01, dy01, s01), s23 = __builtin_elementwise_fma(dy23, dy23, s23);
// ... 1433 lines not shown
```

loam_amd/csrc/register_kernels.hip:

```cpp
#include "loamx_internal.h"

namespace loamx {

namespace {

__device__ __forceinline__ double wave_min(double v) {
#pragma unroll
  for (int off = 32; off >= 1; off >>= 1) v = fmin(v, __shfl_xor(v, off));
  return v;
}
__device__ __forceinline__ double wave_max(double v) {
#pragma unroll
  for (int off = 32; off >= 1; off >>= 1) v = fmax(v, __shfl_xor(v, off));
  return v;
}

#ifndef LOAMX_BUILD_THREADS
#define LOAMX_BUILD_THREADS 1024
#endif
constexpr int kBuildThreads = LOAMX_BUILD_THREADS;

template <bool ORDERED, bool PACKED>
__global__ __launch_bounds__(kBuildThreads) void grid_build_kernel(const double* __restrict__ pts_base,
                                                                   const uint32_t* __restrict__ n_pts, size_t stride,
// ... 899 lines not shown
  __shared__ uint32_t s_rows[(ONE_STAGE ? kLeanRowWords : kLean2RowWords) * kRestThreads];
  const RegKind& K = B.kind[PLANE];
  const RegKindConfig& CK = C.kind[PLANE];
  const size_t stride = K.stride;
  const size_t field = B.n_pairs * stride;
  uint32_t* __restrict__ rnn = K.rnn;
  const uint32_t* __restrict__ rest = K.rest + pair * stride;
  uint32_t* __restrict__ left = K.exact + pair * stride;
  const GridSet &gs = K.grid, &src_gs = K.src_grid;
  const GridDesc g = gs.desc[pair];
  const uint32_t* __restrict__ cs = gs.cell_start + pair * (size_t)(kGridCellsCap + 1);
  const GridPoint* __restrict__ sp = gs.sorted + pair * gs.stride;
  const bool spread = queue_spread(B.n_pairs, queued, blocks_per_pair);
  const uint32_t t0 = spread ? chunk0 + blocks_per_pair * threadIdx.x : chunk0 * kRestThreads + threadIdx.x;
  const uint32_t dt = spread ? 0xFFFFFFFFu - t0 : blocks_per_pair * kRestThreads;
  const bool lean_set = queue_lean_set(g);
  const int kq = CK.k;
  const double max_dist = CK.r, pass_max = CK.pass;
  for (uint32_t t = t0; t < queued; t += dt) {
    const uint32_t entry = rest[t], i = entry & kQueueIndex;
    const size_t slot = pair * stride + t;
    uint32_t pos[KM];
#pragma unroll
    for (int j = 0; j < KM; j++) pos[j] = 0;
    int kept = -1;
    const bool coop = !one_stage && queue_leftovers_coop(C, PLANE);
    if (queue_rest_searches(entry, one_stage, lean_set, coop)) {
      const GridPoint sq = src_gs.sorted[pair * src_gs.stride + i];
      const Vec3 p = pose_act(S.est, v3(sq.x, sq.y, sq.z));
      if (entry & kQueueWide)
        kept = knn_search_f32_round1<KM, true>(g, cs, sp, gs.rel + pair * 3 * gs.stride, (uint32_t)gs.stride, p, kq, max_dist, pass_max, pos,
                                                s_rows + threadIdx.x, kRestThreads);
      else if (!one_stage)
        kept = knn_lean_round2<KM>(g, cs, sp, gs.rel + pair * 3 * gs.stride, (uint32_t)gs.stride, p, kq, max_dist, pass_max, pos,
                                   s_rows + threadIdx.x, kRestThreads);
      if (one_stage && kept < 0)
        kept = knn_search_keyed<KM>(g, cs, sp, p, kq, max_dist, pass_max, pos, s_rows + threadIdx.x, kRestThreads);
    }
    rnn[slot] = (uint32_t)kept;
    if (kept < 0) left[atomicAdd(&B.n_assoc[8 * pair + (PLANE ? 5 : 4)], 1u)] = t;
#pragma unroll
    for (int j = 0; j < KM; j++) rnn[(1 + j) * field + slot] = pos[j];
  }
}

template <bool PLANE, int KM>
__global__ __launch_bounds__(kRestThreads, kLeftWaves) void associate_knn_left_kernel(RegBatch B, RegConfig C,
                                                                                              uint32_t blocks_per_pair) {
  size_t pair;
  uint32_t chunk0;
  if (!assoc_map(B, blockIdx.x, blocks_per_pair, pair, chunk0)) return;
  const PairState& S = B.state[pair];
  if (!S.active) return;
  const uint32_t listed = B.n_assoc[8 * pair + (PLANE ? 5 : 4)];
  if (listed == 0u) return;
  __shared__ uint32_t s_rows[kLeanRowWords * kRestThreads];
  const RegKind& K = B.kind[PLANE];
  const RegKindConfig& CK = C.kind[PLANE];
  const size_t stride = K.stride;
  const size_t field = B.n_pairs * stride;
  uint32_t* __restrict__ rnn = K.rnn;
  const uint32_t* __restrict__ rest = K.rest + pair * stride;
  const uint32_t* __restrict__ left = K.exact + pair * stride;
  const GridSet &gs = K.grid, &src_gs = K.src_grid;
  const GridDesc g = gs.desc[pair];
  const uint32_t* __restrict__ cs = gs.cell_start + pair * (size_t)(kGridCellsCap + 1);
  const GridPoint* __restrict__ sp = gs.sorted + pair * gs.stride;
  const bool spread = queue_spread(B.n_pairs, listed, blocks_per_pair);
  const uint32_t t0 = spread ? chunk0 + blocks_per_pair * threadIdx.x : chunk0 * kRestThreads + threadIdx.x;
  const uint32_t dt = spread ? 0xFFFFFFFFu - t0 : blocks_per_pair * kRestThreads;
  for (uint32_t t = t0; t < listed; t += dt) {
    const uint32_t qpos = left[t], i = rest[qpos] & kQueueIndex;
    const size_t slot = pair * stride + qpos;
    const GridPoint sq = src_gs.sorted[pair * src_gs.stride + i];
    const Vec3 p = pose_act(S.est, v3(sq.x, sq.y, sq.z));
    uint32_t pos[KM];
    const int kept = knn_search_keyed<KM>(g, cs, sp, p, CK.k, CK.r, CK.pass, pos, s_rows + threadIdx.x, kRestThreads);
    rnn[slot] = (uint32_t)kept;
#pragma unroll
    for (int j = 0; j < KM; j++) rnn[(1 + j) * field + slot] = pos[j];
  }
}

constexpr int32_t kCoopMaxShell = 64;

__device__ __forceinline__ double wave_min_all(double v) {
#pragma unroll
  for (int off = 32; off >= 1; off >>= 1) {
    const double o = __shfl_xor(v, off);
    v = knn_key_min(v, o);
  }
  return v;
}

template <int KM>
__device__ __forceinline__ int knn_coop_search(const GridDesc& g, const uint32_t* __restrict__ cell_start, const GridPoint* __restrict__ sp,
                                               Vec3 q, int k, double max_dist, double pass_max, uint32_t pos[KM]) {
  const int lane = threadIdx.x & 63;
#pragma unroll
  for (int j = 0; j < KM; j++) pos[j] = 0;
  if (g.n_points == 0 || k <= 0) return 0;
  if (k > KM) k = KM;
  const int32_t cx = grid_cell_coord(q.x, g.ox, g.inv_h), cy = grid_cell_coord(q.y, g.oy, g.inv_h), cz = grid_cell_coord(q.z, g.oz, g.inv_h);
  const int32_t out = grid_outside_distance(g, cx, cy, cz);
  if (max_dist > 0.0 && out >= 1 && (double)(out - 1) * g.h >= max_dist) return 0;
  int32_t W = 0x7FFFFFFF;
  if (max_dist > 0.0) {
    const double wf = ceil(max_dist * g.inv_h) + 1.0 + (double)out;
    if (wf < 1.0e6) W = (int32_t)wf;
  }
  if (W > kCoopMaxShell) {
    const int32_t span = (g.nx > g.ny ? (g.nx > g.nz ? g.nx : g.nz) : (g.ny > g.nz ? g.ny : g.nz)) + out;
    if (span > kCoopMaxShell) return -2;
    W = span;
  }
  const double r2 = knn_radius_bound(max_dist);
  double bound = r2;
  KnnKeys<KM> c;
  knn_init(c, k, g.n_points);
  bool done = false;
  double kth = knn_key_empty();
  bool fresh = false;
  for (int32_t w = 1; w <= W && !done; w++) {
    const int ring_rows = w == 1 ? 9 : 8 * w;
    const int inner_rows = w == 1 ? 0 : (2 * w - 1) * (2 * w - 1);
    const int pieces = ring_rows + 2 * inner_rows;
    for (int u0 = 0; u0 < pieces; u0 += 64) {
      uint32_t rb = 0, re = 0;
      double s2 = kDblMax;
      {
        const int u = u0 + lane;
        int32_t dy = 0, dz = 0, xlo = cx - w, xhi = cx + w;
        bool cap = false;
        if (w == 1) {
          constexpr int kOrder[9] = {4, 1, 3, 5, 7, 0, 2, 6, 8};
          const int j = kOrder[u < 9 ? u : 0];
          dy = j % 3 - 1, dz = j / 3 - 1;
        } else if (u < ring_rows) {
          const int side = 2 * w + 1, inner = 2 * w - 1;
          if (u < side) dy = u - w, dz = -w;
          else if (u < 2 * side) dy = u - side - w, dz = w;
          else if (u < 2 * side + inner) dy = -w, dz = u - 2 * side - (w - 1);
          else dy = w, dz = u - 2 * side - inner - (w - 1);
        } else {
          const int v = u - ring_rows, ri = v >> 1, inner = 2 * w - 1;
          dy = ri % inner - (w - 1), dz = ri / inner - (w - 1);
          xlo = xhi = (v & 1) ? cx + w : cx - w;
          cap = true;
        }
        const int32_t iy = cy + dy, iz = cz + dz;
        if (u < pieces && iy >= 0 && iy <= g.ny - 1 && iz >= 0 && iz <= g.nz - 1) {
          const double sy = dy == 0 ? 0.0 : slab_dist(q.y, g.oy, g.h, iy), sz = dz == 0 ? 0.0 : slab_dist(q.z, g.oz, g.h, iz);
          double pmin2 = sy * sy + sz * sz;
          if (cap) {
            const double sx = slab_dist(q.x, g.ox, g.h, xlo);
            pmin2 += sx * sx;
          }
          if (pmin2 <= bound) {
            if (!cap) {
              if (xlo < 0) xlo = 0;
              if (xhi > g.nx - 1) xhi = g.nx - 1;
              if (bound < kDblMax) {
                const double reach = sqrt(bound - pmin2) + 1e-9 * g.h;
                const int32_t xl = grid_cell_coord(q.x - reach, g.ox, g.inv_h), xh = grid_cell_coord(q.x + reach, g.ox, g.inv_h);
                if (xl > xlo) xlo = xl;
                if (xh < xhi) xhi = xh;
              }
            }
            if (xlo <= xhi && xlo >= 0 && xhi <= g.nx - 1) {
              const uint32_t row = (uint32_t)((iz * g.ny + iy) * g.nx);
              rb = cell_start_at(cell_start, row + (uint32_t)xlo);
              re = cell_start_at(cell_start, row + (uint32_t)xhi + 1u);
              s2 = pmin2;
            }
          }
        }
      }
      unsigned long long rows = __ballot(rb < re);
      while (rows) {
        const int b = __ffsll(rows) - 1;
        rows &= rows - 1;
        const uint32_t begin = (uint32_t)__builtin_amdgcn_readlane((int)rb, b), end = (uint32_t)__builtin_amdgcn_readlane((int)re, b);
        const double rs2 = __hiloint2double(__builtin_amdgcn_readlane(__double2hiint(s2), b), __builtin_amdgcn_readlane(__double2loint(s2), b));
        if (rs2 > bound) continue;
        fresh = true;
        for (uint32_t p0 = begin; p0 < end; p0 += 64) {
          const uint32_t p = p0 + (uint32_t)lane;
          const bool real = p < end;
          const GridPoint t = sp[real ? p : begin];
          const double dx = q.x - t.x, dy = q.y - t.y, dz = q.z - t.z;
          const double d2 = dx * dx + dy * dy + dz * dz;
          knn_key_insert(c, knn_key_pack(d2, p, c.mask, real));
        }
        if (end - begin >= 256u) {
          const double wb = wave_min_all(knn_bound(c, k));
          bound = wb < bound ? wb : bound;
        }
      }
    }
    {
      if (fresh) {
      fresh = false;
      KnnKeys<KM> cc = c;
      kth = knn_key_empty();
      for (int t = 0; t < k; t++) {
        double head = knn_key_empty();
#pragma unroll
        for (int j = KM; j >= 0; j--)
          if (j >= KM - k) head = cc.key[j] < head ? cc.key[j] : head;
        const double best = wave_min_all(head);
        kth = best;
        if (head == best && best < knn_key_empty()) {
#pragma unroll
          for (int j = 0; j < KM; j++)
            if (j >= KM - k) cc.key[j] = cc.key[j + 1];
          cc.key[KM] = knn_key_empty();
        }
      }
      }
      KnnKeys<KM> probe;
      probe.mask = c.mask;
#pragma unroll
      for (int j = 0; j <= KM; j++) probe.key[j] = kth;
      if (kth < knn_key_empty()) {
        const double ub = knn_bound(probe, k);
        bound = ub < bound ? ub : bound;
      }
      done = knn_done(g, q, k, max_dist, cx, cy, cz, probe, w);
    }
  }
  if (!done) return -1;
  KnnKeys<KM> m;
  knn_init(m, k, g.n_points);
#pragma unroll
  for (int t = 0; t <= KM; t++) {
    if (t >= KM - k) {
      double head = knn_key_empty();
#pragma unroll
      for (int j = KM; j >= 0; j--)
        if (j >= KM - k) head = c.key[j] < head ? c.key[j] : head;
      const double best = wave_min_all(head);
      m.key[t] = best;
      if (head == best && best < knn_key_empty()) {
#pragma unroll
        for (int j = 0; j < KM; j++)
          if (j >= KM - k) c.key[j] = c.key[j + 1];
        c.key[KM] = knn_key_empty();
      }
    }
  }
  return knn_keys_finish(m, k, pass_max, pos);
}

static_assert(kRestThreads == 64, "associate_knn_coop_kernel is written for one wavefront per workgroup");
template <bool PLANE, int KM>
__global__ __launch_bounds__(kRestThreads, LOAMX_COOP_WAVES) void associate_knn_coop_kernel(RegBatch B, RegConfig C, uint32_t blocks_per_pair) {
  size_t pair;
  uint32_t chunk0;
  if (!assoc_map(B, blockIdx.x, blocks_per_pair, pair, chunk0)) return;
  const PairState& S = B.state[pair];
  if (!S.active) return;
  const uint32_t listed = B.n_assoc[8 * pair + (PLANE ? 5 : 4)];
  if (listed == 0u) return;
  __shared__ uint32_t s_rows[kLeanRowWords];
  const RegKind& K = B.kind[PLANE];
  const RegKindConfig& CK = C.kind[PLANE];
  const size_t stride = K.stride;
  const size_t field = B.n_pairs * stride;
  uint32_t* __restrict__ rnn = K.rnn;
  const uint32_t* __restrict__ rest = K.rest + pair * stride;
  const uint32_t* __restrict__ left = K.exact + pair * stride;
  const GridSet &gs = K.grid, &src_gs = K.src_grid;
  const GridDesc g = gs.desc[pair];
  const uint32_t* __restrict__ cs = gs.cell_start + pair * (size_t)(kGridCellsCap + 1);
  const GridPoint* __restrict__ sp = gs.sorted + pair * gs.stride;
  const int kq = CK.k;
  const double max_dist = CK.r, pass_max = CK.pass;
  for (uint32_t t = chunk0; t < listed; t += blocks_per_pair) {
    const uint32_t qpos = left[t], i = rest[qpos] & kQueueIndex;
    const size_t slot = pair * stride + qpos;
    const GridPoint sq = src_gs.sorted[pair * src_gs.stride + i];
    const Vec3 p = pose_act(S.est, v3(sq.x, sq.y, sq.z));
    uint32_t pos[KM];
    int kept = knn_coop_search<KM>(g, cs, sp, p, kq, max_dist, pass_max, pos);
    if (kept == -2) {
      if ((threadIdx.x & 63) == 0) kept = knn_search_keyed<KM>(g, cs, sp, p, kq, max_dist, pass_max, pos, s_rows, 1);
      kept = __builtin_amdgcn_readfirstlane(kept);
#pragma unroll
      for (int j = 0; j < KM; j++) pos[j] = (uint32_t)__builtin_amdgcn_readfirstlane((int)pos[j]);
    }
    if ((threadIdx.x & 63) == 0) {
      rnn[slot] = (uint32_t)kept;
#pragma unroll
      for (int j = 0; j < KM; j++) rnn[(1 + j) * field + slot] = pos[j];
    }
  }
}

template <bool PLANE, int KM>
__device__ __forceinline__ void knn_exact_one(const RegBatch& B, const RegConfig& C, const PairState& S, size_t pair, uint32_t i,
                                              size_t slot, uint32_t* rnn, uint32_t* s_rows, int rows_stride) {
  const RegKind& K = B.kind[PLANE];
  const RegKindConfig& CK = C.kind[PLANE];
  const size_t stride = K.stride;
  const size_t field = B.n_pairs * stride;
  const GridSet &gs = K.grid, &src_gs = K.src_grid;
  const GridDesc g = gs.desc[pair];
  const uint32_t* __restrict__ cs = gs.cell_start + pair * (size_t)(kGridCellsCap + 1);
  const GridPoint* __restrict__ sp = gs.sorted + pair * gs.stride;
  int k = CK.k;
  k = k < KM ? k : KM;
  const GridPoint sq = src_gs.sorted[pair * src_gs.stride + i];
  const Vec3 p = pose_act(S.est, v3(sq.x, sq.y, sq.z));
  KnnResult<KM> r;
  const int kept = knn_search(g, cs, sp, p, k, CK.r, r, s_rows, rows_stride);
  uint32_t pos[KM];
  knn_shift_positions<KM>(r.pos, k, pos);
  rnn[slot] = (uint32_t)kept;
#pragma unroll
  for (int j = 0; j < KM; j++) rnn[(size_t)(1 + j) * field + slot] = pos[j];
}

template <bool PLANE, int KM, bool QUEUED = false, int HANDOFF = 0>
__device__ __forceinline__ bool fit_one(const RegBatch& B, const RegConfig& C, const PairState& S, size_t pair, uint32_t i,
                                        const uint32_t* nnsrc, size_t nidx) {
  const RegKind& K = B.kind[PLANE];
  const RegKindConfig& CK = C.kind[PLANE];
  const size_t stride = K.stride;
  const GridSet &gs = K.grid, &src_gs = K.src_grid;
  const size_t field = B.n_pairs * stride, slot = pair * stride + i;
  const GridPoint sq = src_gs.sorted[pair * src_gs.stride + i];
  const Vec3 p = pose_act(S.est, v3(sq.x, sq.y, sq.z));
  const GridPoint* __restrict__ sp = gs.sorted + pair * gs.stride;
  int kept = (int)nnsrc[nidx];
  const int kq = CK.k;
  const int shift = KM - (kq < KM ? kq : KM);
  double prim[6] = {0, 0, 0, 0, 0, 0};
  uint32_t nearest = 0xFFFFFFFFu;
  bool valid = false;
  uint32_t at[KM];
#pragma unroll
  for (int j = 0; j < KM; j++) at[j] = shift + j < KM ? nnsrc[(size_t)(1 + shift + j) * field + nidx] : 0u;
  if (!QUEUED && kept == -1) return false;
  GridPoint tp[KM];
#pragma unroll
  for (int j = 0; j < KM; j++) tp[j] = sp[at[j] < (uint32_t)gs.stride ? at[j] : 0u];
  if ((HANDOFF & 2) && ((uint32_t)kept & kNnUnverified)) {
    kept = knn_handoff_verify<KM>((uint32_t)kept, p, tp, kq, CK.pass, knn_f32_err_unit(gs.desc[pair]));
    if (kept < 0 || (C.flags & kRegFlagForceLate)) {
      const uint32_t at = atomicAdd(&B.n_assoc[8 * pair + 6 + (PLANE ? 1 : 0)], 1u);
      K.exact[pair * stride + (stride - 1 - at)] = i;
      return false;
    }
    if (B.want_nn_counts) K.nn[nidx] = (uint32_t)kept;
  }
  if (kept >= CK.min_pts) {
    Vec3 nb[KM];
#pragma unroll
    for (int j = 0; j < KM; j++) nb[j] = j < kept ? v3(tp[j].x, tp[j].y, tp[j].z) : v3(0, 0, 0);
    if (kept > 0) nearest = tp[0].orig;
    if (PLANE) {
      Vec3 nrm;
      double d;
      const double avg = fit_plane<KM>(nb, kept, nrm, d);
      valid = !(avg > C.max_avg_plane_dist);
      prim[0] = nrm.x, prim[1] = nrm.y, prim[2] = nrm.z, prim[3] = d;
    } else {
      Vec3 a, b;
      fit_line<KM>(nb, kept, a, b);
      valid = !(kDblMax < C.min_line_cond);
      prim[0] = a.x, prim[1] = a.y, prim[2] = a.z, prim[3] = b.x, prim[4] = b.y, prim[5] = b.z;
    }
  }
  double* __restrict__ rec = K.rec;
  rec[slot] = valid ? p.x : __longlong_as_double(0x7FF8000000000000ll);
  rec[field + slot] = p.y;
  rec[2 * field + slot] = p.z;
#pragma unroll
// ... 1001 lines not shown
  for (int kind = 0; kind < 2; kind++) launch_grid_build_source(B, C, kind, s);
}

void launch_state_init(const RegBatch& B, const RegConfig& C, hipStream_t s) {
  if (B.n_pairs == 0) return;
  launch_kernel(state_init_kernel, dim3(per_pair_grid(B.n_pairs)), dim3(64), 0, s, B, C);
}

#ifndef LOAMX_REST_BLOCKS
#define LOAMX_REST_BLOCKS 32u
#endif
constexpr size_t kQueueTwoStageMin = 16u << 20;
static bool queue_one_stage(const RegBatch& B, const RegConfig& C, int kind) {
  if (C.flags & kRegFlagQueueTwoStage) return false;
  if (C.flags & kRegFlagQueueOneStage) return true;
  if (!(C.flags & kRegFlagNoCoopLeft)) return false;
  return B.n_pairs * B.kind[kind].stride < kQueueTwoStageMin;
}
static uint32_t coop_blocks(size_t n_pairs) {
  const size_t want = 32768 / (n_pairs ? n_pairs : 1);
  return (uint32_t)(want < 32 ? 32 : (want > 4096 ? 4096 : want));
}
static uint32_t rest_blocks(size_t n_pairs, uint32_t nblk) {
  const uint32_t cover = nblk * (uint32_t)(kAssocThreads / kRestThreads);
  uint32_t want = (uint32_t)(4096 / (n_pairs ? n_pairs : 1));
  if (want < LOAMX_REST_BLOCKS) want = LOAMX_REST_BLOCKS;
  return want < cover ? want : cover;
}
void launch_associate(const RegBatch& B, const RegConfig& C, hipStream_t s, hipStream_t aux, hipStream_t aux2, hipEvent_t ev_fork,
                      hipEvent_t ev_mid, hipEvent_t ev_join, hipEvent_t ev_join2, LaunchScope* knn_scope, uint32_t what,
                      AssocCensusRun* census) {
  if (B.n_pairs == 0) return;
  auto census_at = [&](int kind, int stage, hipStream_t st) {
    if (census && census->buf[kind].counts && B.kind[kind].stride)
      launch_kernel(assoc_census_kernel, dim3((unsigned)((B.kind[kind].stride + 255) / 256)), dim3(256), 0, st, B, kind, census->buf[kind], stage);
  };
  AssocCensusRun unread = {};
  AssocCensusForm* const note = census ? census->form : unread.form;
  auto blocks = [](const RegKind& K) { return K.assoc_blocks != 0xFFFFFFFFu ? K.assoc_blocks : (uint32_t)((K.stride + kAssocThreads - 1) / kAssocThreads); };
  const uint32_t be = blocks(B.kind[kEdge]), bp = blocks(B.kind[kPlane]);
  const size_t pair_groups = (B.n_pairs + 7) / 8;
#define LOAMX_ASSOC_A1(PL, KMV, nblk, st)                                                                         \
  do {                                                                                                            \
    const dim3 grid_((unsigned)(pair_groups * 8 * (nblk)));                                                       \
    const uint32_t mode_ = B.kind[PL].knn_mode;                       \
    note[PL].km = (KMV);                                                                                          \
    if (mode_ != 2u) {                                                                                            \
      note[PL].search |= LOAMX_ASSOC_SEARCH_GRID;                                                                 \
      LaunchScope* outer_ = g_launch_scope;                                                                       \
      if ((PL) && knn_scope) g_launch_scope = knn_scope;                                                          \
      launch_kernel((associate_knn_kernel<PL, KMV>), grid_, dim3(kAssocThreads), 0, (st), B, C, (nblk));     \
      g_launch_scope = outer_;                                                                                    \
    }                                                                                                             \
    if (mode_ != 1u) {                                                                                            \
      note[PL].search |= LOAMX_ASSOC_SEARCH_BRUTE;                                                                \
      launch_kernel((associate_knn_brute_kernel<PL, KMV>), grid_, dim3(kAssocThreads), 0, (st), B, C, (nblk)); \
    }                                                                                                             \
    census_at((PL), 0, (st));                                                                                     \
  } while (0)
#define LOAMX_ASSOC_A2(PL, KMV, nblk, st)                                                                         \
  launch_kernel((associate_fit_kernel<PL, KMV>), dim3((unsigned)(pair_groups * 8 * (nblk))), dim3(kAssocThreads), 0, \
                     (st), B, C, (nblk))
#define LOAMX_ASSOC_B(PL, KMV, nblk, st)                                                                          \
  do {                                                                                                            \
    const uint32_t rblk_ = rest_blocks(B.n_pairs, (nblk));                                                        \
    const uint32_t one_ = queue_one_stage(B, C, (PL)) ? 1u : 0u;                                                  \
    note[PL].km = (KMV), note[PL].rest_blocks = rblk_, note[PL].one_stage = one_;                                 \
    if (one_) {                                                                                                   \
      launch_kernel((associate_knn_rest_kernel<PL, KMV, true>), dim3((unsigned)(pair_groups * 8 * rblk_)),   \
                         dim3(kRestThreads), 0, (st), B, C, rblk_);                                               \
      census_at((PL), 1, (st));                                                                                   \
    } else {                                                                                                      \
      launch_kernel((associate_knn_rest_kernel<PL, KMV, false>), dim3((unsigned)(pair_groups * 8 * rblk_)),  \
                         dim3(kRestThreads), 0, (st), B, C, rblk_);                                               \
      census_at((PL), 1, (st));                                                                                   \
      if (!queue_leftovers_coop(C, (PL))) {                                                                       \
        note[PL].leftover_kernel = LOAMX_ASSOC_LEFTOVER_LEFT;                                                     \
        launch_kernel((associate_knn_left_kernel<PL, KMV>), dim3((unsigned)(pair_groups * 8 * rblk_)),       \
                           dim3(kRestThreads), 0, (st), B, C, rblk_);                                             \
      } else {                                                                                                    \
        const uint32_t cblk_ = coop_blocks(B.n_pairs);                                                            \
        note[PL].leftover_kernel = LOAMX_ASSOC_LEFTOVER_COOP, note[PL].coop_blocks = cblk_;                       \
        launch_kernel((associate_knn_coop_kernel<PL, KMV>), dim3((unsigned)(pair_groups * 8 * cblk_)),       \
                           dim3(kRestThreads), 0, (st), B, C, cblk_);                                             \
      }                                                                                                           \
    }                                                                                                             \
    census_at((PL), 2, (st));                                                                                     \
    launch_kernel((associate_fit_queued_kernel<PL, KMV>), dim3((unsigned)(pair_groups * 8 * rblk_)),         \
                       dim3(kRestThreads), 0, (st), B, C, rblk_);                                                 \
  } while (0)
#define LOAMX_ASSOC_K(STEP, PL, nblk, st)                \
  do {                                                   \
    if (C.kind[PL].k <= 5) STEP(PL, 5, nblk, st);        \
    else if (C.kind[PL].k <= 8) STEP(PL, 8, nblk, st);   \
    else STEP(PL, 16, nblk, st);                         \
  } while (0)
  const bool edges = (what & kAssocEdges) != 0u && be != 0u, planes = (what & kAssocPlanes) != 0u && bp != 0u;
  if (edges && planes && B.kind[kEdge].knn_mode == 2u && B.kind[kPlane].knn_mode == 1u && C.kind[kEdge].k <= 5 && C.kind[kPlane].k <= 5 &&
      !(C.flags & kRegFlagNoMixedAssoc)) {
    const uint32_t edge_blocks = (uint32_t)(pair_groups * 8 * be);
    const dim3 grid((unsigned)(edge_blocks + pair_groups * 8 * bp));
    LaunchScope* outer = g_launch_scope;
    if (knn_scope) g_launch_scope = knn_scope;
    launch_kernel((associate_knn_mixed_kernel<5, 5>), grid, dim3(kAssocThreads), 0, s, B, C, be, bp, edge_blocks);
    g_launch_scope = outer;
    note[kEdge].mixed_launch = note[kPlane].mixed_launch = 1u, note[kEdge].km = note[kPlane].km = 5u;
    note[kEdge].search = LOAMX_ASSOC_SEARCH_BRUTE, note[kPlane].search = LOAMX_ASSOC_SEARCH_GRID;
    census_at(kEdge, 0, s), census_at(kPlane, 0, s);
    hipStream_t sb = aux2 ? aux2 : aux;
    const bool fork2 = sb != nullptr && hipEventRecord(ev_mid, s) == hipSuccess && hipStreamWaitEvent(sb, ev_mid, 0) == hipSuccess;
    launch_kernel((associate_fit_mixed_kernel<5, 5>), grid, dim3(kAssocThreads), 0, s, B, C, be, bp, edge_blocks);
    LOAMX_ASSOC_B(true, 5, bp, (fork2 ? sb : s));
    if (fork2 && hipEventRecord(aux2 ? ev_join2 : ev_join, sb) == hipSuccess) (void)hipStreamWaitEvent(s, aux2 ? ev_join2 : ev_join, 0);
    if (LOAMX_HANDOFF & 2) {
      const uint32_t lblk = rest_blocks(B.n_pairs, bp);
      launch_kernel((associate_fit_late_kernel<true, 5>), dim3((unsigned)(pair_groups * 8 * lblk)), dim3(kRestThreads), 0, s, B, C, lblk);
    }
    return;
  }
  const bool use_aux = aux != nullptr && planes;
  const bool fork = use_aux && (edges || !aux2) && hipEventRecord(ev_fork, s) == hipSuccess &&
                    hipStreamWaitEvent(aux, ev_fork, 0) == hipSuccess;
  hipStream_t sa = fork ? aux : s;
  if (edges) {
    LOAMX_ASSOC_K(LOAMX_ASSOC_A1, false, be, sa);
    LOAMX_ASSOC_K(LOAMX_ASSOC_A2, false, be, sa);
    if (B.kind[kEdge].knn_mode != 2u) LOAMX_ASSOC_K(LOAMX_ASSOC_B, false, be, sa);
  }
  if (planes) {
    LOAMX_ASSOC_K(LOAMX_ASSOC_A1, true, bp, s);
    hipStream_t sb = aux2 ? aux2 : aux;
    const bool fork2 = use_aux && (aux2 || fork) && hipEventRecord(ev_mid, s) == hipSuccess && hipStreamWaitEvent(sb, ev_mid, 0) == hipSuccess;
    LOAMX_ASSOC_K(LOAMX_ASSOC_A2, true, bp, s);
    if (B.kind[kPlane].knn_mode != 2u) LOAMX_ASSOC_K(LOAMX_ASSOC_B, true, bp, (fork2 ? sb : s));
    if (fork2 && aux2 && hipEventRecord(ev_join2, aux2) == hipSuccess) (void)hipStreamWaitEvent(s, ev_join2, 0);
  }
  if (fork && hipEventRecord(ev_join, aux) == hipSuccess) (void)hipStreamWaitEvent(s, ev_join, 0);
#undef LOAMX_ASSOC_A1
#undef LOAMX_ASSOC_A2
#undef LOAMX_ASSOC_B
#undef LOAMX_ASSOC_K
}

#ifdef LOAMX_NN_SAME_STATS
__global__ void nn_same_kernel(RegBatch B, uint32_t* prev, unsigned long long* stats, uint32_t it) {
  const size_t pair = blockIdx.y;
  const uint32_t i = blockIdx.x * blockDim.x + threadIdx.x;
  const uint32_t n = B.kind[kPlane].n_src[pair * B.in_pitch];
  if (i >= n || i >= B.kind[kPlane].stride || !B.state[pair].active) return;
  const size_t field = B.n_pairs * B.kind[kPlane].stride, slot = pair * B.kind[kPlane].stride + i;
  bool same = it > 0, queued = B.kind[kPlane].nn[slot] == 0xFFFFFFFFu;
  for (int f = 0; f < 6; f++) {
    const uint32_t v = B.kind[kPlane].nn[f * field + slot];
    if (prev[f * field + slot] != v) same = false;
    prev[f * field + slot] = v;
  }
  atomicAdd(&stats[0], 1ull);
  if (same && !queued) atomicAdd(&stats[1], 1ull);
  if (queued) atomicAdd(&stats[2], 1ull);
}
void debug_nn_same(const RegBatch& B, uint32_t it, hipStream_t s) {
  static uint32_t* prev = nullptr;
  static unsigned long long* stats = nullptr;
  const size_t words = 6 * B.n_pairs * B.kind[kPlane].stride;
  if (!prev) { (void)hipMalloc(&prev, words * 4); (void)hipMalloc(&stats, 24); }
  (void)hipMemsetAsync(stats, 0, 24, s);
  launch_kernel(nn_same_kernel, dim3((unsigned)((B.kind[kPlane].stride + 255) / 256), (unsigned)B.n_pairs), dim3(256), 0, s, B, prev, stats, it);
// ... 45 lines not shown
```

Before: 107,400 pairs/s.

## Split cooperative leftover kNN wavefront into four 16-lane rows per query

The cooperative leftover kNN kernel now processes four queries per wavefront, each searched by a 16-lane row, instead of one query per whole 64-lane wavefront. The search is generalized into a row-width template that uses row-local ballots, bpermute reads and swizzle-based reductions. Queries flagged as wide or tied still take the full-wavefront path. This aims to raise useful lane utilization when queries have small neighborhoods, at the cost of extra shared memory, more divergence and slower per-query progress on dense cells. A census counter of which form was used and an opt-out flag are added.

```diff
diff --git a/include/loamx.h b/include/loamx.h
--- a/include/loamx.h
+++ b/include/loamx.h
@@ -171,6 +171,7 @@
   size_t late_cap;
 } loamx_assoc_census;
 int loamx_ctx_last_assoc_census(loamx_ctx* ctx, int which_kind, loamx_assoc_census* out);
+int loamx_ctx_last_assoc_coop_forms(loamx_ctx* ctx, int which_kind, uint32_t out[2]);
 int loamx_ctx_set_option(loamx_ctx* ctx, const char* name, int value);
 int loamx_ctx_get_option(loamx_ctx* ctx, const char* name, int* value);
 
diff --git a/loam_amd/capi.py b/loam_amd/capi.py
--- a/loam_amd/capi.py
+++ b/loam_amd/capi.py
@@ -254,6 +254,7 @@
     "loamx_comm_info", "loamx_gather_results_dev", "loamx_comm_barrier", "loamx_comm_stats", "loamx_ctx_extract_counters",
     "loamx_ctx_set_option", "loamx_ctx_get_option", "loamx_ctx_last_extract_route", "loamx_ctx_last_solve_census",
     "loamx_ctx_last_assoc_census",
+    "loamx_ctx_last_assoc_coop_forms",
     "loamx_fit_lines", "loamx_fit_planes", "loamx_knn_search", "loamx_associate", "loamx_target_index_stats",
     "loamx_register_scan_sequence_dev", "loamx_register_scan_sequence_dev_f32", "loamx_register_scan_sequence",
     "loamx_register_scan_sequence_f32", "loamx_compose_trajectory_dev", "loamx_deskew_scans_dev", "loamx_deskew_scans_dev_f32",
@@ -469,6 +470,7 @@
     lib.loamx_ctx_last_extract_route.argtypes = [vp, C.POINTER(C.c_uint32)]
     lib.loamx_ctx_last_solve_census.argtypes = [vp, C.c_size_t, C.POINTER(SolveCensusStruct)]
     lib.loamx_ctx_last_assoc_census.argtypes = [vp, C.c_int, C.POINTER(AssocCensusStruct)]
+    lib.loamx_ctx_last_assoc_coop_forms.argtypes = [vp, C.c_int, u32p]
     lib.loamx_registration_information.argtypes = [vp, dp, C.c_size_t, dp, C.c_size_t, dp, C.c_size_t, dp, C.c_size_t, dp,
                                                    C.POINTER(RegistrationParams), C.POINTER(RegInformation)]
     lib.loamx_registration_information_indexed.argtypes = [vp, vp, dp, C.c_size_t, dp, C.c_size_t, dp, C.POINTER(RegistrationParams),
@@ -954,6 +956,12 @@
                            v.edge_stride, v.planar_stride, v.n_se, v.n_sp, v.walk, v.listed_total, v.s0max, v.v2max, v.sweep_chunk,
                            v.edge_cache, v.list_cache, v.flat_cache, counts[:v.live_tiles].copy())
 
+    def last_assoc_coop_forms(self, kind):
+        kind = {"edge": 0, "plane": 1}.get(kind, kind)
+        out = (C.c_uint32 * 2)()
+        self._check(self.lib.loamx_ctx_last_assoc_coop_forms(self.h, kind, out))
+        return int(out[0]), int(out[1])
+
     def last_assoc_census(self, kind):
         kind = {"edge": 0, "plane": 1}.get(kind, kind)
         v = AssocCensusStruct()
diff --git a/loam_amd/csrc/api_core.hip b/loam_amd/csrc/api_core.hip
--- a/loam_amd/csrc/api_core.hip
+++ b/loam_amd/csrc/api_core.hip
@@ -30,7 +30,7 @@
     {"NO_GRID_SIDE", false, kRegFlagNoGridSide}, {"DEBUG_POISON", false, kRegFlagPoison},
     {"QUEUE_TWO_STAGE", false, kRegFlagQueueTwoStage}, {"QUEUE_ONE_STAGE", false, kRegFlagQueueOneStage},
     {"NO_MIXED_ASSOC", false, kRegFlagNoMixedAssoc}, {"FORCE_RCCL", false, kRegFlagForceRccl},
-    {"NO_COOP_LEFT", false, kRegFlagNoCoopLeft}, {"NO_REF_MOMENTS", false, kRegFlagNoRefMoments},
+    {"NO_COOP_LEFT", false, kRegFlagNoCoopLeft}, {"NO_COOP_ROWS", false, kRegFlagNoCoopRows}, {"NO_REF_MOMENTS", false, kRegFlagNoRefMoments},
     {"NO_EXTRACT_BOXES", false, kRegFlagNoExtractBoxes}, {"CHECK_FINITE", false, kRegFlagCheckFinite},
     {"NO_SMALL_SETS", false, kRegFlagNoSmallSets}, {"FORCE_LATE_VERIFY", false, kRegFlagForceLate},
     {"NO_LIVE_DEAL", false, kRegFlagNoLiveDeal}, {"NO_CLOUDMAP_COMBINE", false, kRegFlagNoCloudmapCombine}};
diff --git a/loam_amd/csrc/api_host.h b/loam_amd/csrc/api_host.h
--- a/loam_amd/csrc/api_host.h
+++ b/loam_amd/csrc/api_host.h
@@ -83,6 +83,7 @@
     std::vector<uint32_t> entry;
     std::vector<int32_t> after_rest, before_fit;
     std::vector<uint32_t> late;
+    uint32_t coop_forms[2] = {0, 0};
   } last_assoc_census[2];
   bool last_assoc_census_valid = false;
 
diff --git a/loam_amd/csrc/api_register.hip b/loam_amd/csrc/api_register.hip
--- a/loam_amd/csrc/api_register.hip
+++ b/loam_amd/csrc/api_register.hip
@@ -269,6 +269,7 @@
     c.rest_blocks = F.rest_blocks, c.coop_blocks = F.coop_blocks;
     c.origin[0] = g.ox, c.origin[1] = g.oy, c.origin[2] = g.oz, c.h = g.h, c.nx = g.nx, c.ny = g.ny, c.nz = g.nz, c.n_points = g.n_points;
     c.verified = counts[0], c.unverified = counts[1], c.queued_words = counts[2];
+    keep.coop_forms[0] = counts[5], keep.coop_forms[1] = counts[6];
     c.queued = na[2 + kind], c.listed = na[4 + kind], c.exact = counts[4], c.leftover_finished = counts[3] - counts[4], c.late = na[6 + kind];
     const uint32_t q = c.queued < K.stride ? c.queued : (uint32_t)K.stride;
     keep.entry.assign(q, 0u), keep.after_rest.assign(q, 0), keep.before_fit.assign(q, 0);
@@ -582,6 +583,15 @@
   return LOAMX_OK;
 }
 
+int loamx_ctx_last_assoc_coop_forms(loamx_ctx* ctx, int which_kind, uint32_t out[2]) {
+  if (!out) return LOAMX_ERR_BAD_PARAM;
+  API_LOCK(ctx);
+  if (which_kind != 0 && which_kind != 1) return fail(ctx, LOAMX_ERR_BAD_PARAM, "which_kind: 0 = edges, 1 = planes");
+  if (!ctx->last_assoc_census_valid) return fail(ctx, LOAMX_ERR_BAD_PARAM, "no association dump on this context to read (or another call came after it)");
+  out[0] = ctx->last_assoc_census[which_kind].coop_forms[0], out[1] = ctx->last_assoc_census[which_kind].coop_forms[1];
+  return LOAMX_OK;
+}
+
 int loamx_associate(loamx_ctx* ctx, const double* src_edge, size_t n_se, const double* src_planar, size_t n_sp, const double* tgt_edge,
                     size_t n_te, const double* tgt_planar, size_t n_tp, const double pose[7], const loamx_reg_params* reg,
                     loamx_assoc_dump* out) {
diff --git a/loam_amd/csrc/loamx_internal.h b/loam_amd/csrc/loamx_internal.h
--- a/loam_amd/csrc/loamx_internal.h
+++ b/loam_amd/csrc/loamx_internal.h
@@ -119,6 +119,7 @@
 constexpr uint32_t kRegFlagQueueOneStage = 64u;
 constexpr uint32_t kRegFlagForceRccl = 256u;
 constexpr uint32_t kRegFlagNoCoopLeft = 512u;
+constexpr uint32_t kRegFlagNoCoopRows = 131072u;
 constexpr uint32_t kRegFlagNoRefMoments = 1024u;
 constexpr uint32_t kRegFlagNoSmallSets = 8192u;
 constexpr uint32_t kRegFlagCheckFinite = 4096u;
diff --git a/loam_amd/csrc/reg_math.h b/loam_amd/csrc/reg_math.h
--- a/loam_amd/csrc/reg_math.h
+++ b/loam_amd/csrc/reg_math.h
@@ -807,6 +807,222 @@
   return knn_keys_finish(c, k, pass_max, pos);
 }
 
+constexpr int32_t kCoopMaxShell = 64;
+
+#if defined(__HIP_DEVICE_COMPILE__)
+__device__ __forceinline__ uint32_t row32_xor16_b32(uint32_t v) {
+  return (uint32_t)__builtin_amdgcn_ds_swizzle((int)v, 0x401F);
+}
+template <int J>
+__device__ __forceinline__ double row16_xor_key(double v) {
+  return knn_key_join(row16_xor_b32<J>(knn_key_hi(v)), row16_xor_b32<J>(knn_key_lo(v)));
+}
+#endif
+
+template <int L, int NL>
+LOAMX_HD uint64_t knn_row_ballot(const bool (&flag)[NL], int lane0) {
+#if defined(__HIP_DEVICE_COMPILE__)
+  static_assert(NL == 1, "a device lane holds its own flag");
+  const uint64_t all = __ballot(flag[0]);
+  if constexpr (L == 64) return all;
+  else return (all >> (lane0 & ~(L - 1))) & ((1ull << L) - 1ull);
+#else
+  (void)lane0;
+  uint64_t m = 0;
+  for (int v = 0; v < NL; v++) m |= (uint64_t)flag[v] << v;
+  return m;
+#endif
+}
+template <int L, int NL>
+LOAMX_HD uint32_t knn_row_read(const uint32_t (&word)[NL], int b, int lane0) {
+#if defined(__HIP_DEVICE_COMPILE__)
+  static_assert(NL == 1, "a device lane holds its own word");
+  if constexpr (L == 64) return (uint32_t)__builtin_amdgcn_readlane((int)word[0], b);
+  else return (uint32_t)__builtin_amdgcn_ds_bpermute(((lane0 & ~(L - 1)) + b) << 2, (int)word[0]);
+#else
+  (void)lane0;
+  return word[b];
+#endif
+}
+template <int L, int NL>
+LOAMX_HD double knn_row_key_min(const double (&key)[NL]) {
+  double m = key[0];
+#if defined(__HIP_DEVICE_COMPILE__)
+  static_assert(NL == 1, "a device lane holds its own key");
+  if constexpr (L == 64) {
+#pragma unroll
+    for (int off = 32; off >= 1; off >>= 1) m = knn_key_min(m, __shfl_xor(m, off));
+  } else {
+    m = knn_key_min(m, row16_xor_key<1>(m)), m = knn_key_min(m, row16_xor_key<2>(m));
+    m = knn_key_min(m, row16_xor_key<4>(m)), m = knn_key_min(m, row16_xor_key<8>(m));
+    if constexpr (L == 32) m = knn_key_min(m, knn_key_join(row32_xor16_b32(knn_key_hi(m)), row32_xor16_b32(knn_key_lo(m))));
+  }
+#else
+  for (int v = 1; v < NL; v++) m = knn_key_min(m, key[v]);
+#endif
+  return m;
+}
+
+LOAMX_HD void knn_coop_piece(const GridDesc& g, const uint32_t* __restrict__ cell_start, const Vec3& q, int32_t cx, int32_t cy, int32_t cz,
+                             int32_t w, int u, int ring_rows, int pieces, double bound, uint32_t& rb, uint32_t& re, double& s2) {
+  rb = 0, re = 0, s2 = kDblMax;
+  int32_t dy = 0, dz = 0, xlo = cx - w, xhi = cx + w;
+  bool cap = false;
+  if (w == 1) {
+    constexpr int kOrder[9] = {4, 1, 3, 5, 7, 0, 2, 6, 8};
+    const int j = kOrder[u < 9 ? u : 0];
+    dy = j % 3 - 1, dz = j / 3 - 1;
+  } else if (u < ring_rows) {
+    const int side = 2 * w + 1, inner = 2 * w - 1;
+    if (u < side) dy = u - w, dz = -w;
+    else if (u < 2 * side) dy = u - side - w, dz = w;
+    else if (u < 2 * side + inner) dy = -w, dz = u - 2 * side - (w - 1);
+    else dy = w, dz = u - 2 * side - inner - (w - 1);
+  } else {
+    const int v = u - ring_rows, ri = v >> 1, inner = 2 * w - 1;
+    dy = ri % inner - (w - 1), dz = ri / inner - (w - 1);
+    xlo = xhi = (v & 1) ? cx + w : cx - w;
+    cap = true;
+  }
+  const int32_t iy = cy + dy, iz = cz + dz;
+  if (!(u < pieces && iy >= 0 && iy <= g.ny - 1 && iz >= 0 && iz <= g.nz - 1)) return;
+  const double sy = dy == 0 ? 0.0 : slab_dist(q.y, g.oy, g.h, iy), sz = dz == 0 ? 0.0 : slab_dist(q.z, g.oz, g.h, iz);
+  double pmin2 = sy * sy + sz * sz;
+  if (cap) {
+    const double sx = slab_dist(q.x, g.ox, g.h, xlo);
+    pmin2 += sx * sx;
+  }
+  if (!(pmin2 <= bound)) return;
+  if (!cap) {
+    if (xlo < 0) xlo = 0;
+    if (xhi > g.nx - 1) xhi = g.nx - 1;
+    if (bound < kDblMax) {
+      const double reach = sqrt(bound - pmin2) + 1e-9 * g.h;
+      const int32_t xl = grid_cell_coord(q.x - reach, g.ox, g.inv_h), xh = grid_cell_coord(q.x + reach, g.ox, g.inv_h);
+      if (xl > xlo) xlo = xl;
+      if (xh < xhi) xhi = xh;
+    }
+  }
+  if (xlo <= xhi && xlo >= 0 && xhi <= g.nx - 1) {
+    const uint32_t row = (uint32_t)((iz * g.ny + iy) * g.nx);
+    rb = cell_start_at(cell_start, row + (uint32_t)xlo);
+    re = cell_start_at(cell_start, row + (uint32_t)xhi + 1u);
+    s2 = pmin2;
+  }
+}
+
+template <int KM, int L, int NL>
+LOAMX_HD double knn_row_draw(const KnnKeys<KM> (&c)[NL], double prev) {
+  double head[NL];
+#pragma unroll
+  for (int v = 0; v < NL; v++) {
+    head[v] = knn_key_empty();
+#pragma unroll
+    for (int j = KM; j >= 0; j--) head[v] = c[v].key[j] > prev ? c[v].key[j] : head[v];
+  }
+  return knn_row_key_min<L, NL>(head);
+}
+
+template <int KM, int L, int NL>
+LOAMX_HD int knn_coop_search_rows(const GridDesc& g, const uint32_t* __restrict__ cell_start, const GridPoint* __restrict__ sp, Vec3 q,
+                                  int k, double max_dist, double pass_max, int lane0, uint32_t pos[KM]) {
+  static_assert(L == 16 || L == 32 || L == 64, "a row of 16 lanes, two of them, or the wavefront");
+  static_assert(NL == 1 || NL == L, "the caller holds one lane or the whole row");
+  const int in_row = lane0 & (L - 1);
+#pragma unroll
+  for (int j = 0; j < KM; j++) pos[j] = 0;
+  if (g.n_points == 0 || k <= 0) return 0;
+  if (k > KM) k = KM;
+  const int32_t cx = grid_cell_coord(q.x, g.ox, g.inv_h), cy = grid_cell_coord(q.y, g.oy, g.inv_h), cz = grid_cell_coord(q.z, g.oz, g.inv_h);
+  const int32_t out = grid_outside_distance(g, cx, cy, cz);
+  if (max_dist > 0.0 && out >= 1 && (double)(out - 1) * g.h >= max_dist) return 0;
+  int32_t W = 0x7FFFFFFF;
+  if (max_dist > 0.0) {
+    const double wf = ceil(max_dist * g.inv_h) + 1.0 + (double)out;
+    if (wf < 1.0e6) W = (int32_t)wf;
+  }
+  if (W > kCoopMaxShell) {
+    const int32_t span = (g.nx > g.ny ? (g.nx > g.nz ? g.nx : g.nz) : (g.ny > g.nz ? g.ny : g.nz)) + out;
+    if (span > kCoopMaxShell) return -2;
+    W = span;
+  }
+  const double r2 = knn_radius_bound(max_dist);
+  double bound = r2;
+  KnnKeys<KM> c[NL];
+#pragma unroll
+  for (int v = 0; v < NL; v++) knn_init(c[v], k, g.n_points);
+  bool done = false;
+  double kth = knn_key_empty();
+  bool fresh = false;
+  for (int32_t w = 1; w <= W && !done; w++) {
+    const int ring_rows = w == 1 ? 9 : 8 * w;
+    const int inner_rows = w == 1 ? 0 : (2 * w - 1) * (2 * w - 1);
+    const int pieces = ring_rows + 2 * inner_rows;
+    for (int u0 = 0; u0 < pieces; u0 += L) {
+      uint32_t rb[NL], re[NL], s2hi[NL], s2lo[NL];
+      bool some[NL];
+#pragma unroll
+      for (int v = 0; v < NL; v++) {
+        double s2;
+        knn_coop_piece(g, cell_start, q, cx, cy, cz, w, u0 + in_row + v, ring_rows, pieces, bound, rb[v], re[v], s2);
+        s2hi[v] = knn_key_hi(s2), s2lo[v] = knn_key_lo(s2), some[v] = rb[v] < re[v];
+      }
+      uint64_t turn = knn_row_ballot<L, NL>(some, lane0);
+      while (turn) {
+        const int b = __builtin_ctzll(turn);
+        turn &= turn - 1;
+        const uint32_t begin = knn_row_read<L, NL>(rb, b, lane0), end = knn_row_read<L, NL>(re, b, lane0);
+        const double rs2 = knn_key_join(knn_row_read<L, NL>(s2hi, b, lane0), knn_row_read<L, NL>(s2lo, b, lane0));
+        if (rs2 > bound) continue;
+        fresh = true;
+        for (uint32_t p0 = begin; p0 < end; p0 += (uint32_t)L) {
+#pragma unroll
+          for (int v = 0; v < NL; v++) {
+            const uint32_t p = p0 + (uint32_t)(in_row + v);
+            const bool real = p < end;
+            const GridPoint t = sp[real ? p : begin];
+            const double dx = q.x - t.x, dy = q.y - t.y, dz = q.z - t.z;
+            const double d2 = dx * dx + dy * dy + dz * dz;
+            knn_key_insert(c[v], knn_key_pack(d2, p, c[v].mask, real));
+          }
+        }
+        if (end - begin >= 4u * (uint32_t)L) {
+          double own[NL];
+#pragma unroll
+          for (int v = 0; v < NL; v++) own[v] = knn_bound(c[v], k);
+          const double wb = knn_row_key_min<L, NL>(own);
+          bound = wb < bound ? wb : bound;
+        }
+      }
+    }
+    if (fresh) {
+      fresh = false;
+      kth = -1.0;
+      for (int t = 0; t < k; t++) kth = knn_row_draw<KM, L, NL>(c, kth);
+    }
+    KnnKeys<KM> probe;
+    probe.mask = c[0].mask;
+#pragma unroll
+    for (int j = 0; j <= KM; j++) probe.key[j] = kth;
+    if (kth < knn_key_empty()) {
+      const double ub = knn_bound(probe, k);
+      bound = ub < bound ? ub : bound;
+    }
+    done = knn_done(g, q, k, max_dist, cx, cy, cz, probe, w);
+  }
+  if (!done) return -1;
+  KnnKeys<KM> m;
+  knn_init(m, k, g.n_points);
+  double last = -1.0;
+#pragma unroll
+  for (int t = 0; t <= KM; t++)
+    if (t >= KM - k) m.key[t] = last = knn_row_draw<KM, L, NL>(c, last);
+  return knn_keys_finish(m, k, pass_max, pos);
+}
+
+LOAMX_HD uint32_t knn_coop_deal_first(uint32_t chunk, uint32_t rows) { return chunk * rows; }
+LOAMX_HD uint32_t knn_coop_deal_step(uint32_t blocks, uint32_t rows) { return blocks * rows; }
+
 template <int KM>
 struct KnnKeys32 {
   uint32_t key[KM + 1];
diff --git a/loam_amd/csrc/register_kernels.hip b/loam_amd/csrc/register_kernels.hip
--- a/loam_amd/csrc/register_kernels.hip
+++ b/loam_amd/csrc/register_kernels.hip
@@ -1005,179 +1005,71 @@
   }
 }
 
-constexpr int32_t kCoopMaxShell = 64;
-
-__device__ __forceinline__ double wave_min_all(double v) {
-#pragma unroll
-  for (int off = 32; off >= 1; off >>= 1) {
-    const double o = __shfl_xor(v, off);
-    v = knn_key_min(v, o);
-  }
-  return v;
-}
-
 template <int KM>
 __device__ __forceinline__ int knn_coop_search(const GridDesc& g, const uint32_t* __restrict__ cell_start, const GridPoint* __restrict__ sp,
                                                Vec3 q, int k, double max_dist, double pass_max, uint32_t pos[KM]) {
-  const int lane = threadIdx.x & 63;
-#pragma unroll
-  for (int j = 0; j < KM; j++) pos[j] = 0;
-  if (g.n_points == 0 || k <= 0) return 0;
-  if (k > KM) k = KM;
-  const int32_t cx = grid_cell_coord(q.x, g.ox, g.inv_h), cy = grid_cell_coord(q.y, g.oy, g.inv_h), cz = grid_cell_coord(q.z, g.oz, g.inv_h);
-  const int32_t out = grid_outside_distance(g, cx, cy, cz);
-  if (max_dist > 0.0 && out >= 1 && (double)(out - 1) * g.h >= max_dist) return 0;
-  int32_t W = 0x7FFFFFFF;
-  if (max_dist > 0.0) {
-    const double wf = ceil(max_dist * g.inv_h) + 1.0 + (double)out;
-    if (wf < 1.0e6) W = (int32_t)wf;
-  }
-  if (W > kCoopMaxShell) {
-    const int32_t span = (g.nx > g.ny ? (g.nx > g.nz ? g.nx : g.nz) : (g.ny > g.nz ? g.ny : g.nz)) + out;
-    if (span > kCoopMaxShell) return -2;
-    W = span;
-  }
-  const double r2 = knn_radius_bound(max_dist);
-  double bound = r2;
-  KnnKeys<KM> c;
-  knn_init(c, k, g.n_points);
-  bool done = false;
-  double kth = knn_key_empty();
-  bool fresh = false;
-  for (int32_t w = 1; w <= W && !done; w++) {
-    const int ring_rows = w == 1 ? 9 : 8 * w;
-    const int inner_rows = w == 1 ? 0 : (2 * w - 1) * (2 * w - 1);
-    const int pieces = ring_rows + 2 * inner_rows;
-    for (int u0 = 0; u0 < pieces; u0 += 64) {
-      uint32_t rb = 0, re = 0;
-      double s2 = kDblMax;
-      {
-        const int u = u0 + lane;
-        int32_t dy = 0, dz = 0, xlo = cx - w, xhi = cx + w;
-        bool cap = false;
-        if (w == 1) {
-          constexpr int kOrder[9] = {4, 1, 3, 5, 7, 0, 2, 6, 8};
-          const int j = kOrder[u < 9 ? u : 0];
-          dy = j % 3 - 1, dz = j / 3 - 1;
-        } else if (u < ring_rows) {
-          const int side = 2 * w + 1, inner = 2 * w - 1;
-          if (u < side) dy = u - w, dz = -w;
-          else if (u < 2 * side) dy = u - side - w, dz = w;
-          else if (u < 2 * side + inner) dy = -w, dz = u - 2 * side - (w - 1);
-          else dy = w, dz = u - 2 * side - inner - (w - 1);
-        } else {
-          const int v = u - ring_rows, ri = v >> 1, inner = 2 * w - 1;
-          dy = ri % inner - (w - 1), dz = ri / inner - (w - 1);
-          xlo = xhi = (v & 1) ? cx + w : cx - w;
-          cap = true;
-        }
-        const int32_t iy = cy + dy, iz = cz + dz;
-        if (u < pieces && iy >= 0 && iy <= g.ny - 1 && iz >= 0 && iz <= g.nz - 1) {
-          const double sy = dy == 0 ? 0.0 : slab_dist(q.y, g.oy, g.h, iy), sz = dz == 0 ? 0.0 : slab_dist(q.z, g.oz, g.h, iz);
-          double pmin2 = sy * sy + sz * sz;
-          if (cap) {
-            const double sx = slab_dist(q.x, g.ox, g.h, xlo);
-            pmin2 += sx * sx;
-          }
-          if (pmin2 <= bound) {
-            if (!cap) {
-              if (xlo < 0) xlo = 0;
-              if (xhi > g.nx - 1) xhi = g.nx - 1;
-              if (bound < kDblMax) {
-                const double reach = sqrt(bound - pmin2) + 1e-9 * g.h;
-                const int32_t xl = grid_cell_coord(q.x - reach, g.ox, g.inv_h), xh = grid_cell_coord(q.x + reach, g.ox, g.inv_h);
-                if (xl > xlo) xlo = xl;
-                if (xh < xhi) xhi = xh;
-              }
-            }
-            if (xlo <= xhi && xlo >= 0 && xhi <= g.nx - 1) {
-              const uint32_t row = (uint32_t)((iz * g.ny + iy) * g.nx);
-              rb = cell_start_at(cell_start, row + (uint32_t)xlo);
-              re = cell_start_at(cell_start, row + (uint32_t)xhi + 1u);
-              s2 = pmin2;
-            }
-          }
-        }
-      }
-      unsigned long long rows = __ballot(rb < re);
-      while (rows) {
-        const int b = __ffsll(rows) - 1;
-        rows &= rows - 1;
-        const uint32_t begin = (uint32_t)__builtin_amdgcn_readlane((int)rb, b), end = (uint32_t)__builtin_amdgcn_readlane((int)re, b);
-        const double rs2 = __hiloint2double(__builtin_amdgcn_readlane(__double2hiint(s2), b), __builtin_amdgcn_readlane(__double2loint(s2), b));
-        if (rs2 > bound) continue;
-        fresh = true;
-        for (uint32_t p0 = begin; p0 < end; p0 += 64) {
-          const uint32_t p = p0 + (uint32_t)lane;
-          const bool real = p < end;
-          const GridPoint t = sp[real ? p : begin];
-          const double dx = q.x - t.x, dy = q.y - t.y, dz = q.z - t.z;
-          const double d2 = dx * dx + dy * dy + dz * dz;
-          knn_key_insert(c, knn_key_pack(d2, p, c.mask, real));
-        }
-        if (end - begin >= 256u) {
-          const double wb = wave_min_all(knn_bound(c, k));
-          bound = wb < bound ? wb : bound;
-        }
-      }
-    }
-    {
-      if (fresh) {
-      fresh = false;
-      KnnKeys<KM> cc = c;
-      kth = knn_key_empty();
-      for (int t = 0; t < k; t++) {
-        double head = knn_key_empty();
-#pragma unroll
-        for (int j = KM; j >= 0; j--)
-          if (j >= KM - k) head = cc.key[j] < head ? cc.key[j] : head;
-        const double best = wave_min_all(head);
-        kth = best;
-        if (head == best && best < knn_key_empty()) {
-#pragma unroll
-          for (int j = 0; j < KM; j++)
-            if (j >= KM - k) cc.key[j] = cc.key[j + 1];
-          cc.key[KM] = knn_key_empty();
-        }
-      }
-      }
-      KnnKeys<KM> probe;
-      probe.mask = c.mask;
-#pragma unroll
-      for (int j = 0; j <= KM; j++) probe.key[j] = kth;
-      if (kth < knn_key_empty()) {
-        const double ub = knn_bound(probe, k);
-        bound = ub < bound ? ub : bound;
-      }
-      done = knn_done(g, q, k, max_dist, cx, cy, cz, probe, w);
-    }
-  }
-  if (!done) return -1;
-  KnnKeys<KM> m;
-  knn_init(m, k, g.n_points);
-#pragma unroll
-  for (int t = 0; t <= KM; t++) {
-    if (t >= KM - k) {
-      double head = knn_key_empty();
-#pragma unroll
-      for (int j = KM; j >= 0; j--)
-        if (j >= KM - k) head = c.key[j] < head ? c.key[j] : head;
-      const double best = wave_min_all(head);
-      m.key[t] = best;
-      if (head == best && best < knn_key_empty()) {
-#pragma unroll
-        for (int j = 0; j < KM; j++)
-          if (j >= KM - k) c.key[j] = c.key[j + 1];
-        c.key[KM] = knn_key_empty();
-      }
-    }
-  }
-  return knn_keys_finish(m, k, pass_max, pos);
+  return knn_coop_search_rows<KM, 64, 1>(g, cell_start, sp, q, k, max_dist, pass_max, (int)(threadIdx.x & 63), pos);
 }
 
 static_assert(kRestThreads == 64, "associate_knn_coop_kernel is written for one wavefront per workgroup");
+constexpr int kCoopRowLanes = 16, kCoopRows = 64 / kCoopRowLanes;
+__host__ __device__ inline bool queue_coop_by_rows(const RegConfig& C, const GridDesc& g) {
+  return !(C.flags & kRegFlagNoCoopRows) && queue_lean_set(g);
+}
 template <bool PLANE, int KM>
-__global__ __launch_bounds__(kRestThreads, LOAMX_COOP_WAVES) void associate_knn_coop_kernel(RegBatch B, RegConfig C, uint32_t blocks_per_pair) {
+__device__ __forceinline__ void coop_entry_wave(const RegBatch& B, const RegConfig& C, const PairState& S, size_t pair, const GridDesc& g,
+                                                uint32_t qpos, uint32_t i, uint32_t* s_rows, uint32_t* took) {
+  const RegKind& K = B.kind[PLANE];
+  const RegKindConfig& CK = C.kind[PLANE];
+  const size_t stride = K.stride, field = B.n_pairs * stride;
+  const GridSet &gs = K.grid, &src_gs = K.src_grid;
+  const uint32_t* __restrict__ cs = gs.cell_start + pair * (size_t)(kGridCellsCap + 1);
+  const GridPoint* __restrict__ sp = gs.sorted + pair * gs.stride;
+  uint32_t* __restrict__ rnn = K.rnn;
+  const size_t slot = pair * stride + qpos;
+  const GridPoint sq = src_gs.sorted[pair * src_gs.stride + i];
+  const Vec3 p = pose_act(S.est, v3(sq.x, sq.y, sq.z));
+  uint32_t pos[KM];
+  int kept = knn_coop_search<KM>(g, cs, sp, p, CK.k, CK.r, CK.pass, pos);
+  if (kept == -2) {
+    if ((threadIdx.x & 63) == 0) kept = knn_search_keyed<KM>(g, cs, sp, p, CK.k, CK.r, CK.pass, pos, s_rows, kCoopRows);
+    kept = __builtin_amdgcn_readfirstlane(kept);
+#pragma unroll
+    for (int j = 0; j < KM; j++) pos[j] = (uint32_t)__builtin_amdgcn_readfirstlane((int)pos[j]);
+  }
+  if ((threadIdx.x & 63) == 0) {
+    rnn[slot] = (uint32_t)kept;
+#pragma unroll
+    for (int j = 0; j < KM; j++) rnn[(1 + j) * field + slot] = pos[j];
+    if (took) atomicAdd(&took[1], 1u);
+  }
+}
+template <bool PLANE, int KM>
+__device__ __forceinline__ void coop_entry_row(const RegBatch& B, const RegConfig& C, const PairState& S, size_t pair, const GridDesc& g,
+                                               uint32_t qpos, uint32_t i, uint32_t* s_row, int lane, uint32_t* took) {
+  const RegKind& K = B.kind[PLANE];
+  const RegKindConfig& CK = C.kind[PLANE];
+  const size_t stride = K.stride, field = B.n_pairs * stride;
+  const GridSet &gs = K.grid, &src_gs = K.src_grid;
+  const uint32_t* __restrict__ cs = gs.cell_start + pair * (size_t)(kGridCellsCap + 1);
+  const GridPoint* __restrict__ sp = gs.sorted + pair * gs.stride;
+  uint32_t* __restrict__ rnn = K.rnn;
+  const size_t slot = pair * stride + qpos;
+  const GridPoint sq = src_gs.sorted[pair * src_gs.stride + i];
+  const Vec3 p = pose_act(S.est, v3(sq.x, sq.y, sq.z));
+  uint32_t pos[KM];
+  int kept = knn_coop_search_rows<KM, kCoopRowLanes, 1>(g, cs, sp, p, CK.k, CK.r, CK.pass, lane, pos);
+  if ((lane & (kCoopRowLanes - 1)) == 0) {
+    if (kept == -2) kept = knn_search_keyed<KM>(g, cs, sp, p, CK.k, CK.r, CK.pass, pos, s_row, kCoopRows);
+    rnn[slot] = (uint32_t)kept;
+#pragma unroll
+    for (int j = 0; j < KM; j++) rnn[(1 + j) * field + slot] = pos[j];
+    if (took) atomicAdd(&took[0], 1u);
+  }
+}
+template <bool PLANE, int KM>
+__global__ __launch_bounds__(kRestThreads, LOAMX_COOP_WAVES) void associate_knn_coop_kernel(RegBatch B, RegConfig C, uint32_t blocks_per_pair,
+                                                                                           uint32_t* took) {
   size_t pair;
   uint32_t chunk0;
   if (!assoc_map(B, blockIdx.x, blocks_per_pair, pair, chunk0)) return;
@@ -1185,38 +1077,29 @@
   if (!S.active) return;
   const uint32_t listed = B.n_assoc[8 * pair + (PLANE ? 5 : 4)];
   if (listed == 0u) return;
-  __shared__ uint32_t s_rows[kLeanRowWords];
+  __shared__ uint32_t s_rows[kLeanRowWords * kCoopRows];
   const RegKind& K = B.kind[PLANE];
-  const RegKindConfig& CK = C.kind[PLANE];
   const size_t stride = K.stride;
-  const size_t field = B.n_pairs * stride;
-  uint32_t* __restrict__ rnn = K.rnn;
   const uint32_t* __restrict__ rest = K.rest + pair * stride;
   const uint32_t* __restrict__ left = K.exact + pair * stride;
-  const GridSet &gs = K.grid, &src_gs = K.src_grid;
-  const GridDesc g = gs.desc[pair];
-  const uint32_t* __restrict__ cs = gs.cell_start + pair * (size_t)(kGridCellsCap + 1);
-  const GridPoint* __restrict__ sp = gs.sorted + pair * gs.stride;
-  const int kq = CK.k;
-  const double max_dist = CK.r, pass_max = CK.pass;
-  for (uint32_t t = chunk0; t < listed; t += blocks_per_pair) {
-    const uint32_t qpos = left[t], i = rest[qpos] & kQueueIndex;
-    const size_t slot = pair * stride + qpos;
-    const GridPoint sq = src_gs.sorted[pair * src_gs.stride + i];
-    const Vec3 p = pose_act(S.est, v3(sq.x, sq.y, sq.z));
-    uint32_t pos[KM];
-    int kept = knn_coop_search<KM>(g, cs, sp, p, kq, max_dist, pass_max, pos);
-    if (kept == -2) {
-      if ((threadIdx.x & 63) == 0) kept = knn_search_keyed<KM>(g, cs, sp, p, kq, max_dist, pass_max, pos, s_rows, 1);
-      kept = __builtin_amdgcn_readfirstlane(kept);
-#pragma unroll
-      for (int j = 0; j < KM; j++) pos[j] = (uint32_t)__builtin_amdgcn_readfirstlane((int)pos[j]);
-    }
-    if ((threadIdx.x & 63) == 0) {
-      rnn[slot] = (uint32_t)kept;
-#pragma unroll
-      for (int j = 0; j < KM; j++) rnn[(1 + j) * field + slot] = pos[j];
-    }
+  const GridDesc g = K.grid.desc[pair];
+  if (!queue_coop_by_rows(C, g)) {
+    for (uint32_t t = chunk0; t < listed; t += blocks_per_pair) {
+      const uint32_t qpos = left[t];
+      coop_entry_wave<PLANE, KM>(B, C, S, pair, g, qpos, rest[qpos] & kQueueIndex, s_rows, took);
+    }
+    return;
+  }
+  const int lane = (int)(threadIdx.x & 63), row = lane / kCoopRowLanes;
+  for (uint32_t t0 = knn_coop_deal_first(chunk0, kCoopRows); t0 < listed; t0 += knn_coop_deal_step(blocks_per_pair, kCoopRows)) {
+    for (uint32_t t = t0; t < t0 + kCoopRows && t < listed; t++) {
+      const uint32_t qpos = left[t], entry = rest[qpos];
+      if (entry & (kQueueWide | kQueueTied)) coop_entry_wave<PLANE, KM>(B, C, S, pair, g, qpos, entry & kQueueIndex, s_rows, took);
+    }
+    const uint32_t t = t0 + (uint32_t)row;
+    uint32_t qpos = 0u, entry = kQueueWide;
+    if (t < listed) qpos = left[t], entry = rest[qpos];
+    if (!(entry & (kQueueWide | kQueueTied))) coop_entry_row<PLANE, KM>(B, C, S, pair, g, qpos, entry & kQueueIndex, s_rows + row, lane, took);
   }
 }
 
@@ -2384,7 +2267,8 @@
         const uint32_t cblk_ = coop_blocks(B.n_pairs);                                                            \
         note[PL].leftover_kernel = LOAMX_ASSOC_LEFTOVER_COOP, note[PL].coop_blocks = cblk_;                       \
         launch_kernel((associate_knn_coop_kernel<PL, KMV>), dim3((unsigned)(pair_groups * 8 * cblk_)),       \
-                           dim3(kRestThreads), 0, (st), B, C, cblk_);                                             \
+                           dim3(kRestThreads), 0, (st), B, C, cblk_,                                              \
+                           (census && census->buf[PL].counts) ? census->buf[PL].counts + 5 : (uint32_t*)nullptr);        \
       }                                                                                                           \
     }                                                                                                             \
     census_at((PL), 2, (st));                                                                                     \
```

Result: faster. 109,600 pairs/s, median of 6 (+2.1%).
